# apache/yunikorn-k8shim

Measured on AMD Instinct MI355X. Metric: pod×node predicate evals/sec + decisions/sec, 50k nodes × 1M pods, higher is better.
Workload: dtype int64; 1 GPU; configs[2]: 50k nodes x 1M pods, NodeResourcesFit + TaintToleration + NodeAffinity; nodes_per_gpu=50000, total_nodes=50000, pods=1000000, templates=2000, pod_classes=2061, signature_planes=327, unique_requests=False, spread=False, gang_size=0, parallelism=single GPU

## Files before the change

### yunikorn-k8shim_amd/csrc/engine/engine.hip

```cpp
#include "../../../include/ykpred.h"

#include <hip/hip_runtime.h>
#include <dlfcn.h>
#include <rccl/rccl.h>

#include <algorithm>
#include <chrono>
#include <cstdio>
#include <cstdlib>
#include <cstring>
#include <mutex>
#include <string>
#include <map>
#include <unordered_map>
#include <vector>

#include "kernels.hip.h"
#include "ask_tasks.h"
#include "preempt_headroom_finish.h"

using ykk::i64;
using ykk::u64;

namespace {
// ... 230 lines not shown
  std::vector<uint8_t> vfx_stale;
  int64_t vfx_stale_nodes = 0;
  DevBuf d_pround_live;
  DevBuf d_bytes_gather;
  DevBuf d_topo_agree;
  u64 dict_digest = 0;
  int fuse_rows = 1;
  int fuse_wpl = 0;
  int fuse_count = 0, fuse_row_count = 0;
  bool fuse_ready = false;
  DevBuf d_fuse_rec;
  int fuse_combos = 0;
  int fuse_combine = 1;
  DevBuf d_fuse_combo_rec, d_fuse_combo;
  std::vector<uint8_t> h_class_fused;
  int run_decide = 1;
  int run_ranges = 0, n_decide_list = 0, run_decide_classes = -1;
  bool win_partial = false;
  DevBuf d_run_ranges, d_no_decide, d_glin_r;
  int class_runs = 1;
  int class_runs_min_rows = 16;
  int run_classes = 0, run_units = 0, run_rows = 0;
  DevBuf d_run_classes, d_run_units;
  DevBuf d_sweep_rows, d_sweep_runs, d_sweep_units;
  int sweep_units[ykk::kMaxIdxRows] = {0, 0}, sweep_unit_off[ykk::kMaxIdxRows + 1] = {0, 0, 0};
  DevBuf d_chunk_list_b0;
  int NCB0 = 0;
  DevBuf d_walk2_order, d_walk2_big, d_walk2_begin, d_walk2_len;
  int walk2_chunks = -1;
  DevBuf d_first_r;
  static constexpr bool decide_skip = true;
  DevBuf d_chunk_list_b;
  DevBuf d_slice_general;
  DevBuf d_slice_desc;
  DevBuf d_pfx_r;
  DevBuf d_idx_c;
  DevBuf d_win_r;
  int idx_stride = 0;
  DevBuf d_sig_tol, d_sig_tolflags, d_sig_ports, d_swanted;
  DevBuf d_sig_aff_flags, d_sig_aff_off, d_sig_aff_terms, d_sig_pre_off, d_sig_pre_terms;
  bool specs_set = false;

  int P = 0, C = 0, NC = 0;
  std::vector<int32_t> h_pod_spec, h_pod_pin;
  DevBuf d_pod_spec, d_pod_pin, d_pod_class;
  DevBuf d_class_sig, d_class_pin, d_class_first, d_class_word, d_chunk_class, d_chunk_begin, d_chunk_len, d_chunk_first, d_members;
  std::unordered_map<ClassKey, int32_t, ClassKeyHash> class_ids;
  std::vector<int32_t> h_pod_class, h_pod_slot;
  std::vector<int32_t> h_pod_row;
  int rows_total = 0, rows_a = 0, row_capacity = 0;
  DevBuf d_pod_row;
  bool bands_enabled = true;
  int band_steps = 0;
  int band_steps_now = 128;
  int round_batched = -1;
  int round_node_assume = 1;
  int round_prof = 0;
  int fail_after = 0;
  int sig_wpl = 0;
  int combine_slices = 1;
  int decide_groups_from = 16384;
  int early_counts = 1;
  int group_lds = -1;
  int group_scratch_mb = 256;
  int affinity_fill_waves = 0;
  int group_chunk_tasks = 0;
  int max_lds_bytes = 64 * 1024;
  int num_cus = 256;
  int n_bands = 0, n_band_steps = 0, n_classes_a = 0, n_fix_rows = 0;
  std::vector<int32_t> h_class_slot_a;
  DevBuf d_band_tab, d_class_rows_a, d_class_list_a, d_class_slot_a, d_fix_row, d_fix_slot, d_chunk_zone;
  DevBuf d_class_list_b;
  int n_classes_b = 0;
  std::vector<int32_t> h_ch_zone;
  std::vector<uint8_t> h_row_stale;
  std::vector<int32_t> h_class_sig, h_class_pin, h_class_first, h_class_live;
  std::vector<std::vector<int32_t>> h_class_chunks;
  std::vector<int32_t> h_members, h_ch_class, h_ch_begin, h_ch_len, h_ch_first;
  int patch_chunks = 0;
  bool rank_valid = false;
  uint64_t specs_version = 1, ranked_specs_version = 0, ranked_nodes_epoch = 0;
  unsigned ranked_pre = 0, ranked_filt = 0;
  bool ranked_has_first = false;
  DevBuf d_round;
  DevBuf d_fx_off, d_fx_cls, d_fx_cnt, d_fx_occ, d_sp_sig_of;
  uint64_t fx_version = 0;
  bool fx_contrib = false, fx_ports = false;
  std::vector<int32_t> h_fx_off;
  std::vector<int32_t> h_fx_cls;
  std::vector<int32_t> h_fx_cnt;
  std::vector<uint8_t> h_fx_occupies;
  DevBuf d_patches, d_rows, d_row_count, d_row_best;
  unsigned last_pre = 0, last_filt = 0;
  bool last_eval_valid = false;
  DevBuf d_class_count, d_class_best;
  bool pods_set = false, classes_dirty = true;
  int chunk_members = ykk::kChunkMembers;
  bool chunk_sorted = true;
  int combine_lds_bytes = 40000;

  DevBuf d_bitmap, d_counts, d_decisions, d_keys, d_scratch;
  void* last_bitmap = nullptr;
  int64_t last_bitmap_rows = 0;
  void *last_counts = nullptr, *last_decisions = nullptr, *last_keys = nullptr;

  hipStream_t aux_stream = nullptr;
  hipEvent_t ev_fork = nullptr, ev_planes = nullptr, ev_join = nullptr, ev_counts = nullptr, ev_zero = nullptr;
  hipStream_t peek_stream = nullptr;
  hipEvent_t ev_eval_done = nullptr;
  void* peek_pinned = nullptr;
  size_t peek_pinned_bytes = 0;

  struct GraphKey {
    uint64_t version;
    unsigned pre, filt, options;
    void *bitmap, *counts, *decisions, *keys;
    bool operator==(const GraphKey& o) const {
      return version == o.version && pre == o.pre && filt == o.filt && options == o.options && bitmap == o.bitmap && counts == o.counts &&
             decisions == o.decisions && keys == o.keys;
    }
  };
  std::vector<std::pair<GraphKey, hipGraphExec_t>> graphs;
  std::vector<GraphKey> seen;
  uint64_t tables_version = 1;
  bool graph_disabled = true;

  ncclComm_t comm = nullptr;
  int comm_rank = 0, comm_world = 1, node_offset = 0;
  int64_t round_exchanges = 0;
  void* h_round_pinned = nullptr;
  size_t h_round_pinned_bytes = 0;
  int64_t rounds_batched = 0, round_batched_asks = 0, round_batches = 0, rounds_sequential = 0, round_sequential_asks = 0;
  int forced_stride = 0;
  DevBuf d_gathered, d_gathered_map, d_xkey, d_xcand;
  bool last_has_keys = false;
  DevBuf d_class_rows_all, d_gathered_classes, d_class_rows_slot, d_class_sig_ident, d_expand_count, d_layout_hash, d_gathered_pod_class, d_row_pod;
  int ident_classes = 0;
  uint64_t layout_version = 1, layout_hashed_version = 0, layout_hash_value = 0, row_pod_version = 0;
  uint64_t ask_epoch = 1, hdr_epoch = 0;
  std::vector<uint64_t> hdr_cache;
  uint64_t nodes_epoch = 1, hist_epoch = 0;
  uint64_t bitmap_epoch = 0;

  int64_t n_full_evals = 0, n_node_patches = 0, n_row_patches = 0, n_queries = 0, n_gathers = 0, n_uploads = 0;

  hipEvent_t ev[2 * YKPRED_MAX_TIMED_KERNELS + 2]{};
  bool ev_ready = false;
  int timed = 0;
  const char* timed_name[YKPRED_MAX_TIMED_KERNELS]{};
  bool timing_valid = false;
};

namespace {

int fail(ykpred_engine* e, int code, const std::string& msg) {
  if (e) e->err = msg;
  if (e && (code == YKPRED_E_DEVICE || code == YKPRED_E_NOMEM)) {
    e->last_eval_valid = false;
    e->rank_valid = false;
    e->classes_dirty = true;
    e->spread_dirty = true;
    e->hist_epoch = 0;
    e->ranked_nodes_epoch = 0;
    e->tables_version++;
  }
  return code;
}
inline bool inject_failure(ykpred_engine* e) { return e && e->fail_after > 0 && --e->fail_after == 0; }
#define HIPCHK(call)                                                                                        \
  do {                                                                                                      \
    hipError_t _s = inject_failure(e) ? hipErrorUnknown : (call);                                          \
    if (_s != hipSuccess)                                                                                   \
      return fail(e, _s == hipErrorOutOfMemory ? YKPRED_E_NOMEM : YKPRED_E_DEVICE,                          \
                  std::string(#call) + ": " + hipGetErrorString(_s));                                       \
  } while (0)

template <class T>
int upload(ykpred_engine* e, DevBuf& b, const T* src, size_t n, hipStream_t st) {
  HIPCHK(b.ensure(n * sizeof(T)));
  if (n) HIPCHK(hipMemcpyAsync(b.p, src, n * sizeof(T), hipMemcpyHostToDevice, st));
  return YKPRED_OK;
}
#define TRY(x)                     \
  do {                             \
    int _r = (x);                  \
    if (_r != YKPRED_OK) return _r; \
  } while (0)

ykk::NodeTable node_table(const ykpred_engine* e) {
  ykk::NodeTable t;
  t.n = e->N;
  t.R = e->R;
  t.KT = e->KT;
  t.W = e->W;
  t.alloc = e->d_alloc.as<i64>();
  t.req = e->d_req.as<i64>();
  t.allowed = e->d_allowed.as<int>();
  t.count = e->d_count.as<int>();
  t.flags = e->d_nflags.as<unsigned>();
  t.taints = e->d_taints.as<u64>();
  t.labels = e->d_labels.as<u64>();
  t.KD = e->KD;
  t.KS = e->KS;
  t.domain = e->d_domain.as<int>();
  t.selcount = e->d_selcount.as<int>();
  t.KP = e->KP;
  t.ports = e->d_ports.as<u64>();
  return t;
}
ykk::SpreadSigs spread_sigs(const ykpred_engine* e) {
  ykk::SpreadSigs sp;
  sp.D = e->fam_spread.D;
  sp.c_off = e->d_sp_coff.as<int>();
  sp.c = e->d_sp_c.as<ykk::SpreadC>();
  sp.aff_sig = e->d_sp_aff.as<int>();
  sp.tol_sig = e->d_sp_tol.as<int>();
  sp.cnt = e->d_sp_cnt.as<int>();
  sp.present = e->d_sp_present.as<int>();
  sp.minv = e->d_sp_min.as<int>();
  return sp;
}
ykk::SpecTable spec_table(const ykpred_engine* e) {
  ykk::SpecTable s;
  s.R = e->R;
  s.KT = e->KT;
  s.W = e->W;
  s.req = e->d_sreq.as<i64>();
  s.tol = e->d_stol.as<u64>();
  s.flags = e->d_sflags.as<unsigned>();
  s.aff.flags = e->d_sflags.as<unsigned>();
  s.aff.term_off = e->d_aff_off.as<int>();
  s.aff.terms = e->d_aff_terms.as<u64>();
  s.aff.pre_off = e->d_pre_off.as<int>();
  s.aff.pre_terms = e->d_pre_terms.as<u64>();
  s.KP = e->KP;
  s.wanted_ports = e->d_swanted.as<u64>();
  s.spread_sig = e->d_spec_spread.as<int>();
  s.spread = spread_sigs(e);
  return s;
}

int build_classes(ykpred_engine* e, hipStream_t st) {
  e->tables_version++;
  const int P = e->P;
  auto& ids = e->class_ids;
  ids.clear();
  ids.reserve(1024);
  auto& pod_class = e->h_pod_class;
  pod_class.assign((size_t)P, 0);
  auto &class_sig = e->h_class_sig, &class_pin = e->h_class_pin, &class_size = e->h_class_live;
  class_sig.clear();
  class_pin.clear();
  class_size.clear();
  for (int p = 0; p < P; ++p) {
    int s = e->h_pod_spec[(size_t)p];
    ClassKey k{e->spec_sig_res[(size_t)s], e->spec_sig_tol[(size_t)s], e->spec_sig_aff[(size_t)s], e->spec_sig_spread[(size_t)s],
               e->h_pod_pin[(size_t)p]};
    auto it = ids.find(k);
    int32_t c;
    if (it == ids.end()) {
      c = (int32_t)class_pin.size();
      ids.emplace(k, c);
      class_sig.insert(class_sig.end(), {k.a, k.b, k.c, k.d});
      class_pin.push_back(k.pin);
      class_size.push_back(0);
    } else {
      c = it->second;
    }
    pod_class[(size_t)p] = c;
    class_size[(size_t)c]++;
  }
  const int C = (int)class_pin.size();
  std::vector<int32_t> class_off((size_t)C + 1, 0);
  for (int c = 0; c < C; ++c) class_off[(size_t)c + 1] = class_off[(size_t)c] + class_size[(size_t)c];
  auto& members = e->h_members;
  members.assign((size_t)P, 0);
  e->h_pod_slot.assign((size_t)P, 0);
  std::vector<int32_t> cursor(class_off.begin(), class_off.end() - 1);
  for (int p = 0; p < P; ++p) {
    int slot = cursor[(size_t)pod_class[(size_t)p]]++;
    members[(size_t)slot] = p;
    e->h_pod_slot[(size_t)p] = slot;
  }
  const long row_b = (long)e->row_stride * 8, win = (long)ykk::kBandGroups * 4096;
  const int KC = ykk::kBandClasses;
  auto piece_min_of = [&](int steps) { return (int)((double)steps * (4096.0 + (double)row_b) / (double)row_b / (double)(KC - 1) * 1.3) + 3; };
  int S = e->band_steps;
  if (S <= 0) {
    int s_min = 8;
    while (s_min < 128 && (long)s_min * 4096 < 5L * KC * row_b) s_min *= 2;
    auto coverage = [&](int steps) {
      const int need = 2 * piece_min_of(steps);
      long rows = 0;
      for (int c = 0; c < C; ++c)
        if (class_size[(size_t)c] >= need) rows += class_size[(size_t)c];
      return rows;
    };
    const long best = coverage(s_min);
    S = 128;
    while (S > s_min && (double)coverage(S) < 0.5 * (double)best) S /= 2;
  }
  while (S > 4 && (long)S * win / row_b >= (1L << 21)) S -= 4;
  e->band_steps_now = S;
  const int piece_min = piece_min_of(S);
  e->h_class_slot_a.assign((size_t)C, -1);
  e->h_pod_row.assign((size_t)P, -1);
  std::vector<ykk::BandEntry> band_tab;
  std::vector<int32_t> class_list_a, fix_row, fix_slot;
  int n_steps = 0, n_bands = 0, rows_a = 0;
  const bool geometry_ok = e->bands_enabled && e->N > 0 && (size_t)2 * KC * (size_t)row_b <= (size_t)std::min(ykk::kBandMaxLds, e->max_lds_bytes);
  if (geometry_ok) {
    long rows_needed = 0;
    for (int c = 0; c < C; ++c)
      if (class_size[(size_t)c] >= 2 * piece_min) {
        e->h_class_slot_a[(size_t)c] = (int32_t)class_list_a.size();
        class_list_a.push_back(c);
        rows_needed += class_size[(size_t)c];
      }
    if (rows_needed < (long)S * win / row_b / 4) {
      class_list_a.clear();
      std::fill(e->h_class_slot_a.begin(), e->h_class_slot_a.end(), -1);
    }
  }
  if (!class_list_a.empty()) {
    struct Piece {
      int32_t x, s, slot;
// ... 491 lines not shown
  if (e->row_capacity && e->rows_total > e->row_capacity)
    return fail(e, YKPRED_E_INVALID, "the bitmap needs more rows than ykpred_set_row_capacity allows");
  const int cm = e->chunk_members;
  struct Chunk {
    int32_t cls, begin, len, first, first_row;
  };
  std::vector<Chunk> chunks;
  for (int c = 0; c < C; ++c)
    for (int b = class_off[(size_t)c]; b < class_off[(size_t)c + 1]; b += cm)
      chunks.push_back({c, b, std::min(cm, class_off[(size_t)c + 1] - b), b == class_off[(size_t)c] ? 1 : 0, e->h_pod_row[(size_t)members[(size_t)b]]});
  if (e->chunk_sorted)
    std::stable_sort(chunks.begin(), chunks.end(), [](const Chunk& x, const Chunk& y) { return x.first_row < y.first_row; });
  auto &ch_class = e->h_ch_class, &ch_begin = e->h_ch_begin, &ch_len = e->h_ch_len, &ch_first = e->h_ch_first;
  ch_class.clear();
  ch_begin.clear();
  ch_len.clear();
  ch_first.clear();
  e->h_ch_zone.clear();
  e->h_class_chunks.assign((size_t)C, {});
  for (const Chunk& k : chunks) {
    e->h_class_chunks[(size_t)k.cls].push_back((int32_t)ch_class.size());
    ch_class.push_back(k.cls);
    ch_begin.push_back(k.begin);
    ch_len.push_back(k.len);
    ch_first.push_back(k.first);
    e->h_ch_zone.push_back(e->h_class_slot_a[(size_t)k.cls] >= 0 ? 1 : (e->h_class_sweep[(size_t)k.cls] ? 2 : (e->h_class_fused[(size_t)k.cls] ? 3 : 0)));
  }
  std::vector<int32_t> chunk_list_b;
  for (size_t k = 0; k < e->h_ch_zone.size(); ++k)
    if (e->h_ch_zone[k] != 1) chunk_list_b.push_back((int32_t)k);
  e->NCB = (int)chunk_list_b.size();
  {
    std::vector<int32_t> chunk_list_b0;
    for (size_t k = 0; k < e->h_ch_zone.size(); ++k)
      if (e->h_ch_zone[k] == 0) chunk_list_b0.push_back((int32_t)k);
    e->NCB0 = (int)chunk_list_b0.size();
    TRY(upload(e, e->d_chunk_list_b0, chunk_list_b0.data(), chunk_list_b0.size(), st));
  }
  e->h_class_first.assign((size_t)C, -1);
  for (int c = 0; c < C; ++c) e->h_class_first[(size_t)c] = members[(size_t)class_off[(size_t)c]];
  std::vector<int32_t> member_rows((size_t)P);
  for (int i = 0; i < P; ++i) member_rows[(size_t)i] = e->h_pod_row[(size_t)members[(size_t)i]];
  e->h_row_stale.assign((size_t)P, 0);
  e->C = C;
  e->NC = (int)ch_class.size();
  e->patch_chunks = 0;
  TRY(upload(e, e->d_pod_class, pod_class.data(), pod_class.size(), st));
  TRY(upload(e, e->d_class_sig, class_sig.data(), class_sig.size(), st));
  TRY(upload(e, e->d_class_pin, class_pin.data(), class_pin.size(), st));
  TRY(upload(e, e->d_class_first, e->h_class_first.data(), e->h_class_first.size(), st));
  TRY(upload(e, e->d_members, member_rows.data(), member_rows.size(), st));
  TRY(upload(e, e->d_pod_row, e->h_pod_row.data(), e->h_pod_row.size(), st));
  TRY(upload(e, e->d_chunk_zone, e->h_ch_zone.data(), e->h_ch_zone.size(), st));
  TRY(upload(e, e->d_chunk_list_b, chunk_list_b.data(), chunk_list_b.size(), st));
  TRY(upload(e, e->d_band_tab, band_tab.data(), band_tab.size(), st));
  TRY(upload(e, e->d_class_list_a, class_list_a.data(), class_list_a.size(), st));
  TRY(upload(e, e->d_class_slot_a, e->h_class_slot_a.data(), e->h_class_slot_a.size(), st));
  TRY(upload(e, e->d_fix_row, fix_row.data(), fix_row.size(), st));
  TRY(upload(e, e->d_fix_slot, fix_slot.data(), fix_slot.size(), st));
  HIPCHK(e->d_class_rows_a.ensure((size_t)std::max<size_t>(class_list_a.size(), 1) * (size_t)e->row_stride * sizeof(u64)));
  TRY(upload(e, e->d_chunk_class, ch_class.data(), ch_class.size(), st));
  TRY(upload(e, e->d_chunk_begin, ch_begin.data(), ch_begin.size(), st));
  TRY(upload(e, e->d_chunk_len, ch_len.data(), ch_len.size(), st));
  TRY(upload(e, e->d_chunk_first, ch_first.data(), ch_first.size(), st));
  HIPCHK(e->d_class_count.ensure((size_t)std::max(C, 1) * sizeof(int)));
  HIPCHK(e->d_class_best.ensure((size_t)std::max(C, 1) * sizeof(int)));
  HIPCHK(hipStreamSynchronize(st));
  e->classes_dirty = false;
  e->layout_version++;
  e->last_eval_valid = false;
  return YKPRED_OK;
}

int ensure_planes(ykpred_engine* e, hipStream_t st) {
  int rows = 0;
  for (Family* f : {&e->fam_res, &e->fam_spread, &e->fam_tol, &e->fam_aff}) {
    f->base = rows;
    rows += std::max(f->D, 1);
  }
  size_t need = ((size_t)rows * (size_t)e->row_stride + 64) * sizeof(u64);
  for (DevBuf* b : {&e->planes_canon, &e->planes_ranked}) {
    if (b->cap < need || e->plane_rows_alloc != rows) {
      e->tables_version++;
      HIPCHK(b->ensure(need));
      HIPCHK(hipMemsetAsync(b->p, 0, need, st));
    }
  }
  e->plane_rows_alloc = rows;
  size_t base_need = (size_t)(64 * (e->W + e->KT + e->KP) + 2) * (size_t)e->row_stride * sizeof(u64);
  for (DevBuf* b : {&e->base_canon, &e->base_ranked}) {
    if (b->cap < base_need) {
      e->tables_version++;
      HIPCHK(b->ensure(base_need));
      HIPCHK(hipMemsetAsync(b->p, 0, base_need, st));
    }
  }
  return YKPRED_OK;
}

int build_spread_tables(ykpred_engine* e, hipStream_t st) {
  e->tables_version++;
  std::vector<int32_t> coff{0}, aff, tol;
  std::vector<ykk::SpreadC> rows;
  int64_t cells = 0;
  for (size_t d = 0; d < e->spread_sig.size(); ++d) {
    for (const ykpred_spread_t& c : e->spread_sig[d]) {
      if (c.topology_key < 0 || c.topology_key >= e->KD || c.selector_class >= e->KS)
        return fail(e, YKPRED_E_INVALID, "spread constraint references a topology key / selector class outside the node table");
      ykk::SpreadC r;
      r.kd = c.topology_key;
      r.ks = c.selector_class;
      r.max_skew = c.max_skew;
      r.min_domains = c.min_domains;
      r.self_match = c.self_match;
      r.flags = c.flags;
      r.kind = c.kind;
      r.dom_size = (size_t)c.topology_key < e->h_domain_sizes.size() ? e->h_domain_sizes[(size_t)c.topology_key] : 0;
      r.cnt_off = (int)cells;
      cells += r.dom_size;
      if (cells > 0x7fffffff) return fail(e, YKPRED_E_UNSUPPORTED, "spread histograms exceed 2^31 cells");
      rows.push_back(r);
    }
    coff.push_back((int32_t)rows.size());
    aff.push_back(e->spread_sig_aff[d]);
    tol.push_back(e->spread_sig_tol[d]);
  }
  e->spread_constraints = (int)rows.size();
  e->spread_cells = cells;
  TRY(upload(e, e->d_sp_coff, coff.data(), coff.size(), st));
  TRY(upload(e, e->d_sp_c, rows.data(), rows.size(), st));
  TRY(upload(e, e->d_sp_aff, aff.data(), aff.size(), st));
  TRY(upload(e, e->d_sp_tol, tol.data(), tol.size(), st));
  {
    std::vector<int32_t> sig_of;
    for (size_t d = 0; d < e->spread_sig.size(); ++d) sig_of.insert(sig_of.end(), e->spread_sig[d].size(), (int32_t)d);
    sig_of.resize(std::max<size_t>(rows.size(), 1), 0);
    TRY(upload(e, e->d_sp_sig_of, sig_of.data(), sig_of.size(), st));
  }
  HIPCHK(e->d_sp_cnt.ensure((size_t)std::max<int64_t>(cells, 1) * sizeof(int)));
  HIPCHK(e->d_sp_present.ensure((size_t)std::max<int64_t>(cells, 1) * sizeof(int)));
  HIPCHK(e->d_sp_min.ensure((size_t)std::max(e->spread_constraints, 1) * sizeof(int)));
  HIPCHK(hipStreamSynchronize(st));
  e->spread_dirty = false;
  return YKPRED_OK;
}

struct Timer {
  ykpred_engine* e;
  bool on;
  void start(hipStream_t st) {
    e->timed = 0;
    e->timing_valid = false;
    if (on) (void)hipEventRecord(e->ev[2 * YKPRED_MAX_TIMED_KERNELS], st);
  }
  void begin(hipStream_t st) {
    if (on && e->timed < YKPRED_MAX_TIMED_KERNELS) (void)hipEventRecord(e->ev[2 * e->timed], st);
  }
  void end(hipStream_t st, const char* name) {
    if (trace_kernels_on()) {
      const hipError_t s = hipStreamSynchronize(st);
      fprintf(stderr, "ykpred: %s %s\n", name, s == hipSuccess ? "done" : hipGetErrorString(s));
      fflush(stderr);
    }
    if (!on || e->timed >= YKPRED_MAX_TIMED_KERNELS) return;
    (void)hipEventRecord(e->ev[2 * e->timed + 1], st);
    e->timed_name[e->timed] = name;
    e->timed++;
  }
  void done(hipStream_t st) {
    if (on) (void)hipEventRecord(e->ev[2 * YKPRED_MAX_TIMED_KERNELS + 1], st);
    e->timing_valid = on;
  }
};

int grow_owned_outputs(ykpred_engine* e) {
// ... 237 lines not shown
    g_create_error = "ABI version mismatch";
    return YKPRED_E_INVALID;
  }
  if (cfg->num_resources < 3 || cfg->num_resources > ykk::kMaxR || cfg->taint_words < 1 || cfg->taint_words > ykk::kMaxKT ||
      cfg->label_words < 1 || cfg->label_words > ykk::kMaxWTotal) {
    g_create_error = "config out of range: need 3<=R<=8, 1<=KT<=4, 1<=W<=32";
    return YKPRED_E_UNSUPPORTED;
  }
  if (cfg->topology_keys < 0 || cfg->topology_keys > ykk::kMaxKD || cfg->selector_classes < 0 || cfg->selector_classes > 4096 ||
      cfg->port_words < 0 || cfg->port_words > ykk::kMaxKP) {
    g_create_error = "config out of range: need 0<=KD<=8 topology keys, 0<=KS<=4096 selector classes, 0<=KP<=4 port words";
    return YKPRED_E_UNSUPPORTED;
  }
  int ndev = 0;
  hipError_t s = hipGetDeviceCount(&ndev);
  if (s != hipSuccess || ndev <= 0) {
    g_create_error = std::string("no HIP device: ") + hipGetErrorString(s) + " (libykpred has no CPU fallback)";
    return YKPRED_E_DEVICE;
  }
  if (cfg->device < 0 || cfg->device >= ndev) {
    g_create_error = "device ordinal out of range";
    return YKPRED_E_INVALID;
  }
  s = hipSetDevice(cfg->device);
  if (s != hipSuccess) {
    g_create_error = std::string("hipSetDevice: ") + hipGetErrorString(s);
    return YKPRED_E_DEVICE;
  }
  auto* e = new ykpred_engine();
  e->cfg = *cfg;
  e->R = cfg->num_resources;
  e->KT = cfg->taint_words;
  e->W = cfg->label_words;
  e->KD = cfg->topology_keys;
  e->KS = cfg->selector_classes;
  e->KP = cfg->port_words;
  if (cfg->reserved[0] >= 1 && cfg->reserved[0] <= ykk::kChunkMembers) e->chunk_members = cfg->reserved[0];
  e->chunk_sorted = cfg->reserved[1] != 1;
  if (cfg->reserved[2] > 0 && cfg->reserved[2] <= 160 * 1024) e->combine_lds_bytes = cfg->reserved[2];
  if (cfg->reserved[2] < 0) e->combine_lds_bytes = 0;
  if (cfg->reserved[4] > 0) e->walk_rows = cfg->reserved[4];
  if (cfg->reserved[5] > 0) e->wave_combine_below = cfg->reserved[5];
  if (cfg->reserved[5] < 0) e->wave_combine_below = 0;
  if (cfg->reserved[6] < 0) e->bands_enabled = false;
  if (cfg->reserved[6] > 0) e->band_steps = std::min(256, std::max(4, (cfg->reserved[6] + 3) / 4 * 4));
  e->graph_disabled = cfg->reserved[3] != 1;
  {
    int lds = 0;
    if (hipDeviceGetAttribute(&lds, hipDeviceAttributeMaxSharedMemoryPerBlock, cfg->device) == hipSuccess && lds > 0) e->max_lds_bytes = lds;
    int cus = 0;
    if (hipDeviceGetAttribute(&cus, hipDeviceAttributeMultiprocessorCount, cfg->device) == hipSuccess && cus > 0) e->num_cus = cus;
  }
  if (const char* tune = getenv("YKPRED_TUNE")) {
    std::string text(tune);
    size_t at = 0;
    while (at < text.size()) {
      size_t stop = text.find(',', at);
      if (stop == std::string::npos) stop = text.size();
      const std::string item = text.substr(at, stop - at);
      at = stop + 1;
      if (item.empty()) continue;
      const size_t eq = item.find('=');
      const std::string key = item.substr(0, eq);
      const int val = eq == std::string::npos ? 1 : atoi(item.c_str() + eq + 1);
      if (key == "walk_rows") e->walk_rows = std::max(val, 1);
      else if (key == "sig_wpl") e->sig_wpl = val;
      else if (key == "combine_slices") e->combine_slices = val;
      else if (key == "decide_groups_from") e->decide_groups_from = val;
      else if (key == "graph") e->graph_disabled = val != 1;
      else if (key == "early_counts") e->early_counts = val;
      else if (key == "band_steps") {
        e->bands_enabled = val >= 0;
        e->band_steps = val > 0 ? std::min(256, std::max(4, (val + 3) / 4 * 4)) : 0;
      } else if (key == "chunk_members") e->chunk_members = std::min(std::max(val, 1), (int)ykk::kChunkMembers);
      else if (key == "wave_combine_below") e->wave_combine_below = std::max(val, 0);
      else if (key == "fail_after") e->fail_after = std::max(val, 0);
      else if (key == "round_prof") e->round_prof = val;
      else if (key == "round_batched") e->round_batched = val;
      else if (key == "round_node_assume") e->round_node_assume = val;
      else if (key == "sweep_min_run") e->sweep_min_run = std::max(val, 0);
      else if (key == "sweep_groups") e->sweep_groups = std::max(val, 0);
      else if (key == "class_runs") e->class_runs = val;
      else if (key == "run_decide") e->run_decide = val;
      else if (key == "fuse_rows") e->fuse_rows = val;
      else if (key == "fuse_wpl") e->fuse_wpl = val;
      else if (key == "fuse_combine") e->fuse_combine = val;
      else if (key == "class_runs_min_rows") e->class_runs_min_rows = std::max(val, 1);
      else if (key == "group_lds") e->group_lds = val;
      else if (key == "group_scratch_mb") e->group_scratch_mb = std::max(val, 0);
      else if (key == "group_chunk_tasks") e->group_chunk_tasks = std::max(val, 0);
      else if (key == "affinity_fill_waves") e->affinity_fill_waves = val;
      else {
        g_create_error = "YKPRED_TUNE: unknown key '" + key + "'";
        delete e;
        return YKPRED_E_INVALID;
      }
    }
  }
  s = hipStreamCreateWithFlags(&e->own_stream, hipStreamNonBlocking);
  if (s != hipSuccess) {
    g_create_error = std::string("hipStreamCreate: ") + hipGetErrorString(s);
    delete e;
    return YKPRED_E_DEVICE;
  }
  {
    int lo = 0, hi = 0;
    (void)hipDeviceGetStreamPriorityRange(&lo, &hi);
    if (hipStreamCreateWithPriority(&e->aux_stream, hipStreamNonBlocking, hi) != hipSuccess)
      (void)hipStreamCreateWithFlags(&e->aux_stream, hipStreamNonBlocking);
  }
  if (hipStreamCreateWithFlags(&e->peek_stream, hipStreamNonBlocking) != hipSuccess) e->peek_stream = nullptr;
  (void)hipEventCreateWithFlags(&e->ev_eval_done, hipEventDisableTiming);
  (void)hipEventCreateWithFlags(&e->ev_fork, hipEventDisableTiming);
  (void)hipEventCreateWithFlags(&e->ev_join, hipEventDisableTiming);
  (void)hipEventCreateWithFlags(&e->ev_planes, hipEventDisableTiming);
  (void)hipEventCreateWithFlags(&e->ev_counts, hipEventDisableTiming);
  (void)hipEventCreateWithFlags(&e->ev_zero, hipEventDisableTiming);
  for (auto& ev : e->ev) (void)hipEventCreate(&ev);
  e->ev_ready = true;
  *out = e;
  return YKPRED_OK;
}

void ykpred_destroy(ykpred_engine_t* e) {
  if (!e) return;
  (void)hipSetDevice(e->cfg.device);
  (void)hipDeviceSynchronize();
  if (e->comm) (void)rccl()->CommDestroy(e->comm);
  e->comm = nullptr;
  for (DevBuf* b : {&e->d_gathered, &e->d_gathered_map, &e->d_xkey, &e->d_xcand}) b->release();
  for (auto& g : e->graphs) (void)hipGraphExecDestroy(g.second);
  e->graphs.clear();
  for (DevBuf* b : {&e->d_alloc, &e->d_req, &e->d_allowed, &e->d_count, &e->d_nflags, &e->d_taints, &e->d_labels, &e->d_domain, &e->d_selcount, &e->d_ports, &e->d_sig_ports, &e->d_swanted,
                    &e->d_sp_cnt_prev, &e->d_sp_present_prev, &e->d_sp_min_prev, &e->d_sig_changed, &e->d_class_dirty,
                    &e->d_spec_spread, &e->d_sp_coff, &e->d_sp_c, &e->d_sp_aff, &e->d_sp_tol, &e->d_sp_cnt, &e->d_sp_present, &e->d_sp_min,
                    &e->planes_canon, &e->planes_ranked, &e->base_canon, &e->base_ranked, &e->d_rankbuf, &e->d_score, &e->d_key,
                    &e->d_rank, &e->d_perm, &e->d_sreq, &e->d_stol, &e->d_sflags, &e->d_aff_off, &e->d_aff_terms, &e->d_pre_off,
                    &e->d_pre_terms, &e->d_dim_val, &e->d_dim_order, &e->d_dim_chunk_dim, &e->d_dim_chunk_begin, &e->d_dim_chunk_len,
                    &e->d_res_rows, &e->d_big_dim, &e->d_walk_big, &e->d_walk_begin, &e->d_walk_len, &e->d_sfree_c, &e->d_pmask_c,
                    &e->d_sfree_r, &e->d_pmask_r, &e->d_rbits_c, &e->d_sorted, &e->d_sorted_off, &e->d_ent_c, &e->d_agree, &e->d_topo_agree, &e->d_bytes_gather, &e->d_fuse_rec, &e->d_fuse_combo_rec, &e->d_fuse_combo, &e->d_run_ranges, &e->d_no_decide, &e->d_glin_r, &e->d_run_classes, &e->d_run_units, &e->d_sweep_rows, &e->d_sweep_runs, &e->d_sweep_units, &e->d_chunk_list_b0, &e->d_walk2_order, &e->d_walk2_big, &e->d_walk2_begin, &e->d_walk2_len, &e->d_idx_c, &e->d_win_r, &e->d_pfx_r, &e->d_slice_desc, &e->d_slice_general, &e->d_chunk_list_b, &e->d_first_r, &e->d_sig_tol, &e->d_sig_tolflags, &e->d_sig_aff_flags, &e->d_sig_aff_off,
                    &e->d_sig_aff_terms, &e->d_sig_pre_off, &e->d_sig_pre_terms, &e->d_pod_spec, &e->d_pod_pin, &e->d_pod_class,
                    &e->d_class_sig, &e->d_class_pin, &e->d_class_first, &e->d_class_word, &e->d_chunk_class, &e->d_chunk_begin, &e->d_chunk_len, &e->d_chunk_first,
                    &e->d_pod_row, &e->d_band_tab, &e->d_class_rows_a, &e->d_class_list_a, &e->d_class_slot_a, &e->d_fix_row, &e->d_fix_slot, &e->d_chunk_zone,
                    &e->d_members, &e->d_patches, &e->d_rows, &e->d_row_count, &e->d_row_best, &e->d_class_count, &e->d_class_best, &e->d_bitmap, &e->d_counts, &e->d_decisions, &e->d_keys, &e->d_scratch,
                    &e->d_member_key, &e->d_name_rank, &e->d_member_tie, &e->d_class_rows_all, &e->d_gathered_classes, &e->d_class_rows_slot,
                    &e->d_class_sig_ident, &e->d_expand_count, &e->d_layout_hash, &e->d_gathered_pod_class, &e->d_row_pod,
                    &e->d_round, &e->d_fx_off, &e->d_fx_cls, &e->d_fx_cnt, &e->d_fx_occ, &e->d_sp_sig_of, &e->d_class_list_b, &e->d_gathered, &e->d_gathered_map,
                    &e->d_xkey, &e->d_xcand, &e->d_query, &e->d_groups, &e->d_domain_head, &e->d_rc_req, &e->d_rc_pods, &e->d_rc_ports,
                    &e->d_vt_base, &e->d_vt_tier_end, &e->d_vt_cum, &e->d_vt_ports, &e->d_pround})
    b->release();
  if (e->ev_ready)
    for (auto& ev : e->ev) (void)hipEventDestroy(ev);
  if (e->ev_fork) (void)hipEventDestroy(e->ev_fork);
  if (e->ev_join) (void)hipEventDestroy(e->ev_join);
  if (e->ev_planes) (void)hipEventDestroy(e->ev_planes);
  if (e->ev_counts) (void)hipEventDestroy(e->ev_counts);
  if (e->ev_zero) (void)hipEventDestroy(e->ev_zero);
  if (e->h_round_pinned) (void)hipHostFree(e->h_round_pinned);
  if (e->ev_eval_done) (void)hipEventDestroy(e->ev_eval_done);
  if (e->peek_pinned) (void)hipHostFree(e->peek_pinned);
  if (e->peek_stream) (void)hipStreamDestroy(e->peek_stream);
  if (e->aux_stream) (void)hipStreamDestroy(e->aux_stream);
  if (e->own_stream) (void)hipStreamDestroy(e->own_stream);
  delete e;
}

int32_t ykpred_set_nodes(ykpred_engine_t* e, const ykpred_nodes_t* n) {
  YK_SERIALISE(e);
  Range roctx_range("ykpred:upload_nodes");
  if (e) e->n_uploads++;
  if (e) e->tables_version++;
  if (e) e->nodes_epoch++;
  if (e) e->ask_epoch++;
  if (e) e->last_eval_valid = false;
  if (!e || !n || n->count < 0) return fail(e, YKPRED_E_INVALID, "set_nodes: bad argument");
  if (n->count > 0 && (!n->allocatable || !n->requested || !n->allowed_pods || !n->pod_count || !n->flags || !n->taint_bits ||
                       !n->label_bits))
    return fail(e, YKPRED_E_INVALID, "set_nodes: null column");
  if ((e->KD > 0 && (!n->domain_sizes || (n->count > 0 && !n->domain_id))) || (e->KS > 0 && n->count > 0 && !n->selector_count))
    return fail(e, YKPRED_E_INVALID, "set_nodes: topology / selector columns missing (config has KD/KS > 0)");
  if (e->KP > 0 && n->count > 0 && !n->port_bits) return fail(e, YKPRED_E_INVALID, "set_nodes: port_bits missing (config has KP > 0)");
  HIPCHK(hipSetDevice(e->cfg.device));
  hipStream_t st = e->own_stream;
  e->rank_valid = false;
  const size_t N = (size_t)n->count;
  TRY(upload(e, e->d_alloc, n->allocatable, N * (size_t)e->R, st));
  TRY(upload(e, e->d_req, n->requested, N * (size_t)e->R, st));
  TRY(upload(e, e->d_allowed, n->allowed_pods, N, st));
  TRY(upload(e, e->d_count, n->pod_count, N, st));
  TRY(upload(e, e->d_nflags, n->flags, N, st));
  TRY(upload(e, e->d_taints, n->taint_bits, N * (size_t)e->KT, st));
  TRY(upload(e, e->d_labels, n->label_bits, N * (size_t)e->W, st));
  TRY(upload(e, e->d_domain, n->domain_id, N * (size_t)e->KD, st));
  TRY(upload(e, e->d_selcount, n->selector_count, N * (size_t)e->KS, st));
  TRY(upload(e, e->d_ports, n->port_bits, N * (size_t)e->KP, st));
  e->has_name_rank = n->name_rank != nullptr && N > 0;
  if (e->has_name_rank) TRY(upload(e, e->d_name_rank, n->name_rank, N, st));
  HIPCHK(e->d_member_tie.ensure(std::max<size_t>(N, 1) * sizeof(int)));
  for (int k = 0; k < ykk::kMaxKT; ++k) e->taint_used[k] = 0;
  for (int k = 0; k < e->KT; ++k)
    for (size_t i = 0; i < N; ++i) e->taint_used[k] |= n->taint_bits[(size_t)k * N + i];
  e->h_domain_sizes.assign(n->domain_sizes, n->domain_sizes + e->KD);
  e->spread_dirty = true;
  HIPCHK(e->d_score.ensure(N * sizeof(double)));
  HIPCHK(e->d_key.ensure(N * sizeof(u64)));
  HIPCHK(e->d_rank.ensure(N * sizeof(int)));
  HIPCHK(e->d_perm.ensure(N * sizeof(int)));
  HIPCHK(e->d_rankbuf.ensure((3 * (size_t)ykk::kRankBuckets + 1 + N) * sizeof(int)));
  HIPCHK(e->d_member_key.ensure(N * sizeof(u64)));
  HIPCHK(hipStreamSynchronize(st));
  if (e->N != n->count) {
    e->planes_canon.release();
    e->planes_ranked.release();
    e->base_canon.release();
    e->base_ranked.release();
    e->rc_tiers = 0;
    e->vt_tiers = 0;
    e->vfx_columns = -1;
  }
  e->N = n->count;
  e->row_words = (e->N + 63) / 64;
  e->row_stride = std::max(16, (e->row_words + 15) / 16 * 16);
  if (e->forced_stride) {
    if (e->forced_stride < e->row_stride) return fail(e, YKPRED_E_INVALID, "set_nodes: ykpred_set_row_stride is smaller than this shard needs");
    e->row_stride = e->forced_stride;
  }
  e->nodes_set = true;
  return YKPRED_OK;
}

int32_t ykpred_update_node(ykpred_engine_t* e, int32_t idx, const ykpred_nodes_t* n) {
  YK_SERIALISE(e);
  Range roctx_range("ykpred:update_node");
  if (e) e->n_uploads++;
  if (e) e->tables_version++;
  if (!e || !n || n->count != 1) return fail(e, YKPRED_E_INVALID, "update_node: count must be 1");
  if (!e->nodes_set || idx < 0 || idx >= e->N) return fail(e, YKPRED_E_INVALID, "update_node: index out of range");
  for (int k = 0; k < e->KD; ++k)
    if (n->domain_id[k] >= e->h_domain_sizes[(size_t)k]) return fail(e, YKPRED_E_INVALID, "update_node: new topology domain — re-upload the node table");
  e->nodes_epoch++;
  HIPCHK(hipSetDevice(e->cfg.device));
  hipStream_t st = e->own_stream;
  e->rank_valid = false;
  const size_t N = (size_t)e->N;
  for (int r = 0; r < e->R; ++r) {
    HIPCHK(hipMemcpyAsync(e->d_alloc.as<i64>() + (size_t)r * N + idx, n->allocatable + r, sizeof(i64), hipMemcpyHostToDevice, st));
    HIPCHK(hipMemcpyAsync(e->d_req.as<i64>() + (size_t)r * N + idx, n->requested + r, sizeof(i64), hipMemcpyHostToDevice, st));
  }
  HIPCHK(hipMemcpyAsync(e->d_allowed.as<int>() + idx, n->allowed_pods, sizeof(int), hipMemcpyHostToDevice, st));
  HIPCHK(hipMemcpyAsync(e->d_count.as<int>() + idx, n->pod_count, sizeof(int), hipMemcpyHostToDevice, st));
  HIPCHK(hipMemcpyAsync(e->d_nflags.as<unsigned>() + idx, n->flags, sizeof(unsigned), hipMemcpyHostToDevice, st));
  for (int k = 0; k < e->KT; ++k) {
    e->taint_used[k] |= n->taint_bits[k];
    HIPCHK(hipMemcpyAsync(e->d_taints.as<u64>() + (size_t)k * N + idx, n->taint_bits + k, sizeof(u64), hipMemcpyHostToDevice, st));
  }
  for (int w = 0; w < e->W; ++w)
    HIPCHK(hipMemcpyAsync(e->d_labels.as<u64>() + (size_t)w * N + idx, n->label_bits + w, sizeof(u64), hipMemcpyHostToDevice, st));
  for (int k = 0; k < e->KD; ++k) {
    HIPCHK(hipMemcpyAsync(e->d_domain.as<int>() + (size_t)k * N + idx, n->domain_id + k, sizeof(int), hipMemcpyHostToDevice, st));
  }
  for (int k = 0; k < e->KS; ++k)
    HIPCHK(hipMemcpyAsync(e->d_selcount.as<int>() + (size_t)k * N + idx, n->selector_count + k, sizeof(int), hipMemcpyHostToDevice, st));
  for (int k = 0; k < e->KP; ++k)
    HIPCHK(hipMemcpyAsync(e->d_ports.as<u64>() + (size_t)k * N + idx, n->port_bits + k, sizeof(u64), hipMemcpyHostToDevice, st));
  if (e->has_name_rank && n->name_rank)
    HIPCHK(hipMemcpyAsync(e->d_name_rank.as<int>() + idx, n->name_rank, sizeof(int), hipMemcpyHostToDevice, st));
  HIPCHK(hipStreamSynchronize(st));
  return YKPRED_OK;
}

int32_t ykpred_update_label_word(ykpred_engine_t* e, int32_t word, const uint64_t* column) {
  YK_SERIALISE(e);
  if (!e || !column || word < 0 || word >= (e ? e->W : 0)) return fail(e, YKPRED_E_INVALID, "update_label_word: bad argument");
  if (!e->nodes_set) return fail(e, YKPRED_E_STATE, "update_label_word: no node table");
  e->tables_version++;
  HIPCHK(hipSetDevice(e->cfg.device));
  if (e->N) {
    HIPCHK(hipMemcpyAsync(e->d_labels.as<u64>() + (size_t)word * (size_t)e->N, column, (size_t)e->N * sizeof(u64), hipMemcpyHostToDevice, e->own_stream));
    HIPCHK(hipStreamSynchronize(e->own_stream));
  }
  return YKPRED_OK;
}

int32_t ykpred_set_specs(ykpred_engine_t* e, const ykpred_specs_t* s) {
  YK_SERIALISE(e);
  Range roctx_range("ykpred:upload_specs");
  if (e) e->n_uploads++;
  if (e) e->tables_version++;
  if (e) e->ask_epoch++;
  if (e) e->specs_version++;
  if (!e || !s || s->count < 0) return fail(e, YKPRED_E_INVALID, "set_specs: bad argument");
  if (s->count > 0 && (!s->requests || !s->tolerated || !s->flags || !s->aff_term_off || !s->pre_term_off))
    return fail(e, YKPRED_E_INVALID, "set_specs: null column");
  if (s->spread_off && s->count > 0 && s->spread_off[s->count] != 0 && !s->spread)
    return fail(e, YKPRED_E_INVALID, "set_specs: spread_off without spread rows");
  HIPCHK(hipSetDevice(e->cfg.device));
  hipStream_t st = e->own_stream;
  const int S = s->count, R = e->R, KT = e->KT, W = e->W, KP = e->KP;
  if (KP > 0 && S > 0 && !s->wanted_ports) return fail(e, YKPRED_E_INVALID, "set_specs: wanted_ports missing (config has KP > 0)");
  const int T = S ? s->aff_term_off[S] : 0, M = S ? s->pre_term_off[S] : 0;
  if (T < 0 || M < 0 || (T > 0 && !s->aff_terms) || (M > 0 && !s->pre_terms)) return fail(e, YKPRED_E_INVALID, "set_specs: bad term tables");
  const int oldS = e->S, old_spread_D = e->fam_spread.D;
  bool append_only = e->specs_set && !e->classes_dirty && oldS <= S;
  if (append_only && oldS > 0) {
    auto same = [](const void* a, const void* b, size_t n) { return n == 0 || memcmp(a, b, n) == 0; };
    const int oT = e->h_aff_off[(size_t)oldS], oM = e->h_pre_off[(size_t)oldS];
    append_only = same(e->h_req.data(), s->requests, (size_t)oldS * R * sizeof(i64)) &&
                  same(e->h_tol.data(), s->tolerated, (size_t)oldS * KT * sizeof(u64)) &&
                  (KP == 0 || same(e->h_wanted.data(), s->wanted_ports, (size_t)oldS * KP * sizeof(u64))) &&
                  same(e->h_sflags.data(), s->flags, (size_t)oldS * sizeof(uint32_t)) &&
                  same(e->h_aff_off.data(), s->aff_term_off, (size_t)(oldS + 1) * sizeof(int32_t)) &&
                  same(e->h_pre_off.data(), s->pre_term_off, (size_t)(oldS + 1) * sizeof(int32_t)) &&
                  same(e->h_aff_terms.data(), s->aff_terms, (size_t)oT * W * sizeof(u64)) &&
                  same(e->h_pre_terms.data(), s->pre_terms, (size_t)oM * W * sizeof(u64));
    const bool had_spread = !e->h_spread_off.empty() && e->h_spread_off[(size_t)oldS] > 0;
    if (append_only && (had_spread || s->spread_off)) {
      if (e->h_spread_off.empty() || !s->spread_off) {
        append_only = !had_spread && s->spread_off && s->spread_off[oldS] == 0;
      } else {
        append_only = same(e->h_spread_off.data(), s->spread_off, (size_t)(oldS + 1) * sizeof(int32_t)) &&
                      same(e->h_spread.data(), s->spread, (size_t)e->h_spread_off[(size_t)oldS] * sizeof(ykpred_spread_t));
      }
    }
  }
  if (s->spread_off && S > 0) {
    e->h_spread_off.assign(s->spread_off, s->spread_off + S + 1);
    e->h_spread.assign(s->spread, s->spread + s->spread_off[S]);
  } else {
    e->h_spread_off.assign((size_t)S + 1, 0);
    e->h_spread.clear();
  }
  e->S = S;
  e->h_req.assign(s->requests, s->requests + (size_t)S * R);
  e->h_tol.assign(s->tolerated, s->tolerated + (size_t)S * KT);
  if (KP > 0) e->h_wanted.assign(s->wanted_ports, s->wanted_ports + (size_t)S * KP); else e->h_wanted.clear();
  TRY(upload(e, e->d_swanted, e->h_wanted.data(), e->h_wanted.size(), st));
  e->h_sflags.assign(s->flags, s->flags + S);
  e->h_aff_off.assign(s->aff_term_off, s->aff_term_off + S + (S ? 1 : 0));
  e->h_pre_off.assign(s->pre_term_off, s->pre_term_off + S + (S ? 1 : 0));
  if (!S) {
    e->h_aff_off.assign(1, 0);
    e->h_pre_off.assign(1, 0);
  }
  e->h_aff_terms.assign(s->aff_terms, s->aff_terms + (size_t)T * W);
  e->h_pre_terms.assign(s->pre_terms, s->pre_terms + (size_t)M * W);
  TRY(upload(e, e->d_sreq, e->h_req.data(), e->h_req.size(), st));
  TRY(upload(e, e->d_stol, e->h_tol.data(), e->h_tol.size(), st));
  TRY(upload(e, e->d_sflags, e->h_sflags.data(), e->h_sflags.size(), st));
  TRY(upload(e, e->d_aff_off, e->h_aff_off.data(), e->h_aff_off.size(), st));
  TRY(upload(e, e->d_pre_off, e->h_pre_off.data(), e->h_pre_off.size(), st));
  TRY(upload(e, e->d_aff_terms, e->h_aff_terms.data(), e->h_aff_terms.size(), st));
  TRY(upload(e, e->d_pre_terms, e->h_pre_terms.data(), e->h_pre_terms.size(), st));

  e->spec_sig_res.assign((size_t)S, 0);
  e->spec_sig_tol.assign((size_t)S, 0);
  e->spec_sig_aff.assign((size_t)S, 0);
  std::unordered_map<std::string, int32_t> m_tol, m_aff;
  auto mix64 = [](u64 z) {
    z = (z ^ (z >> 30)) * 0xbf58476d1ce4e5b9ull;
    z = (z ^ (z >> 27)) * 0x94d049bb133111ebull;
    return z ^ (z >> 31);
  };
  size_t tab_cap = 64;
  while (tab_cap < (size_t)S * 2 + 2) tab_cap <<= 1;
  std::vector<int32_t> res_tab(tab_cap, -1);
  std::vector<int32_t> res_first;
  std::vector<std::vector<int32_t>> dim_tab((size_t)R);
  std::vector<size_t> dim_used((size_t)R, 0);
  auto dim_row = [&](int r, i64 q) -> int32_t {
    std::vector<int32_t>& tab = dim_tab[(size_t)r];
    if (tab.empty()) tab.assign(1024, -1);
    if ((dim_used[(size_t)r] + 1) * 2 > tab.size()) {
      std::vector<int32_t> bigger(tab.size() * 4, -1);
// ... 152 lines not shown
      std::vector<int32_t> big_of_dim((size_t)R, 0);
      for (size_t b = 0; b < big_dim.size(); ++b) big_of_dim[(size_t)big_dim[b]] = (int32_t)b + 1;
      for (int32_t& r : res_rows)
        if (r > 0 && big_of_dim[(size_t)e->h_dim_of[(size_t)r]]) r |= big_of_dim[(size_t)e->h_dim_of[(size_t)r]] << ykk::kRowBigShift;
    }
    e->index_rows = 0;
    for (int32_t len : wlen) e->index_rows += len;
    e->h_res_rows = res_rows;
    e->h_row_pos.assign((size_t)rows, -1);
    e->h_row_big.assign((size_t)rows, -1);
    e->sweep_ready = false;
    e->h_sorted_off.assign(1, 0);
    {
      std::vector<i64> sorted;
      for (size_t b = 0; b < big_dim.size(); ++b) {
        const int g = big_dim[b] + 1, b0 = start[(size_t)g], b1 = start[(size_t)g + 1];
        for (int i = b0; i < b1; ++i) {
          e->h_row_pos[(size_t)order[(size_t)i]] = i - b0;
          e->h_row_big[(size_t)order[(size_t)i]] = (int32_t)b;
          sorted.push_back(e->h_dim_val[(size_t)order[(size_t)i]]);
        }
        e->h_sorted_off.push_back((int32_t)sorted.size());
      }
      sorted.push_back(0);
      TRY(upload(e, e->d_sorted, sorted.data(), sorted.size(), st));
      TRY(upload(e, e->d_sorted_off, e->h_sorted_off.data(), e->h_sorted_off.size(), st));
    }
    e->h_stage_rows.clear();
    {
      std::vector<uint8_t> walked((size_t)R, 0);
      for (int32_t d : big_dim) walked[(size_t)d] = 1;
      for (int d = 1; d < rows && (int)e->h_stage_rows.size() < ykk::kWalkMaxStage; ++d)
        if (!walked[(size_t)e->h_dim_of[(size_t)d]]) e->h_stage_rows.push_back(d);
    }
    e->dim_chunks = (int)cdim.size();
    e->n_big = (int)big_dim.size();
    e->walk_chunks = (int)wbig.size();
    TRY(upload(e, e->d_dim_val, e->h_dim_val.data(), e->h_dim_val.size(), st));
    TRY(upload(e, e->d_dim_order, order.data(), order.size(), st));
    TRY(upload(e, e->d_dim_chunk_dim, cdim.data(), cdim.size(), st));
    TRY(upload(e, e->d_dim_chunk_begin, cbegin.data(), cbegin.size(), st));
    TRY(upload(e, e->d_dim_chunk_len, clen.data(), clen.size(), st));
    TRY(upload(e, e->d_big_dim, big_dim.data(), big_dim.size(), st));
    TRY(upload(e, e->d_walk_big, wbig.data(), wbig.size(), st));
    TRY(upload(e, e->d_walk_begin, wbegin.data(), wbegin.size(), st));
    TRY(upload(e, e->d_walk_len, wlen.data(), wlen.size(), st));
    TRY(upload(e, e->d_res_rows, res_rows.data(), res_rows.size(), st));
  }
  TRY(upload(e, e->d_sig_tol, sig_tol.data(), sig_tol.size(), st));
  TRY(upload(e, e->d_sig_tolflags, sig_tolflags.data(), sig_tolflags.size(), st));
  TRY(upload(e, e->d_sig_ports, sig_ports.data(), sig_ports.size(), st));
  TRY(upload(e, e->d_sig_aff_flags, sig_aff_flags.data(), sig_aff_flags.size(), st));
  TRY(upload(e, e->d_sig_aff_off, sig_aff_off.data(), sig_aff_off.size(), st));
  TRY(upload(e, e->d_sig_pre_off, sig_pre_off.data(), sig_pre_off.size(), st));
  TRY(upload(e, e->d_sig_aff_terms, sig_aff_terms.data(), sig_aff_terms.size(), st));
  TRY(upload(e, e->d_sig_pre_terms, sig_pre_terms.data(), sig_pre_terms.size(), st));
  HIPCHK(hipStreamSynchronize(st));
  e->specs_set = true;
  if (!append_only) e->classes_dirty = true;
  if (!spread_unchanged) e->last_eval_valid = false;
  return YKPRED_OK;
}

int32_t ykpred_set_pods(ykpred_engine_t* e, const ykpred_pods_t* p) {
  YK_SERIALISE(e);
  Range roctx_range("ykpred:upload_asks");
  if (e) e->n_uploads++;
  if (e) e->tables_version++;
  if (e) e->ask_epoch++;
  if (!e || !p || p->count < 0) return fail(e, YKPRED_E_INVALID, "set_pods: bad argument");
  if (p->count > 0 && (!p->spec_index || !p->node_name_index)) return fail(e, YKPRED_E_INVALID, "set_pods: null column");
  HIPCHK(hipSetDevice(e->cfg.device));
  e->P = p->count;
  e->h_pod_spec.assign(p->spec_index, p->spec_index + p->count);
  e->h_pod_pin.assign(p->node_name_index, p->node_name_index + p->count);
  TRY(upload(e, e->d_pod_spec, e->h_pod_spec.data(), e->h_pod_spec.size(), e->own_stream));
  TRY(upload(e, e->d_pod_pin, e->h_pod_pin.data(), e->h_pod_pin.size(), e->own_stream));
  HIPCHK(hipStreamSynchronize(e->own_stream));
  e->pods_set = true;
  e->classes_dirty = true;
  return YKPRED_OK;
}

static int validate_state(ykpred_engine* e) {
  if (!e->nodes_set || !e->specs_set || !e->pods_set) return fail(e, YKPRED_E_STATE, "nodes, specs and pods must be uploaded first");
  for (int p = 0; p < e->P; ++p) {
    int s = e->h_pod_spec[(size_t)p], pin = e->h_pod_pin[(size_t)p];
    if (s < 0 || s >= e->S) return fail(e, YKPRED_E_INVALID, "pod references a spec that was not uploaded");
    if (pin < YKPRED_UNKNOWN_NODE_NAME || pin >= e->N) return fail(e, YKPRED_E_INVALID, "pod node_name_index out of range");
  }
  return YKPRED_OK;
}

int32_t ykpred_eval(ykpred_engine_t* e, const ykpred_eval_args_t* a) {
  YK_SERIALISE(e);
  Range roctx_range("ykpred:eval");
  if (!e || !a) return fail(e, YKPRED_E_INVALID, "eval: bad argument");
  HIPCHK(hipSetDevice(e->cfg.device));
  hipStream_t st = a->stream ? (hipStream_t)a->stream : e->own_stream;
  if (e->classes_dirty) {
    if (a->options & (YKPRED_EVAL_SKIP_BITMAP | YKPRED_EVAL_DIRTY_CLASSES))
      return fail(e, YKPRED_E_STATE, "eval: the pod classes are due for a rebuild — run a full ykpred_eval (bitmap included)");
    TRY(validate_state(e));
    TRY(build_classes(e, e->own_stream));
  }
  const unsigned pre = a->prefilter_plugins, filt = a->filter_plugins;
  const bool spread_filt = filt & YKPRED_PLUGIN_POD_TOPOLOGY_SPREAD, spread_pre = pre & YKPRED_PLUGIN_POD_TOPOLOGY_SPREAD;
  const bool ipa_filt = filt & YKPRED_PLUGIN_INTER_POD_AFFINITY, ipa_pre = pre & YKPRED_PLUGIN_INTER_POD_AFFINITY;
  const bool spread_err = (spread_filt && !spread_pre) || (ipa_filt && !ipa_pre) ||
                          ((filt & YKPRED_PLUGIN_NODE_PORTS) && !(pre & YKPRED_PLUGIN_NODE_PORTS));
  if (e->spread_dirty) TRY(build_spread_tables(e, e->own_stream));
  const bool pts_en = spread_filt && spread_pre, ipa_en = ipa_filt && ipa_pre;
  const bool spread_on = (pts_en || ipa_en) && e->fam_spread.D > 0;
  const int N = e->N, P = e->P;
  const size_t bitmap_bytes = (size_t)std::max(std::max(e->rows_total, e->row_capacity), 1) * (size_t)e->row_stride * sizeof(u64);
  u64* bitmap = (u64*)a->bitmap;
  int64_t bitmap_rows = 0;
  if (!bitmap || (void*)bitmap == e->d_bitmap.p) {
    HIPCHK(e->d_bitmap.ensure(bitmap_bytes));
    bitmap = e->d_bitmap.as<u64>();
    bitmap_rows = (int64_t)(e->d_bitmap.cap / ((size_t)std::max(e->row_stride, 1) * sizeof(u64)));
  } else {
    bitmap_rows = a->bitmap_rows ? (int64_t)a->bitmap_rows : (int64_t)e->row_capacity;
    if (bitmap_rows == 0)
      return fail(e, YKPRED_E_INVALID, "eval: a caller-owned bitmap needs eval_args.bitmap_rows or ykpred_set_row_capacity (it must hold layout.num_rows rows)");
    if ((int64_t)e->rows_total > bitmap_rows)
      return fail(e, YKPRED_E_INVALID, "eval: the caller-owned bitmap holds fewer rows than the layout needs (layout.num_rows)");
  }
  e->last_bitmap = bitmap;
  e->last_bitmap_rows = bitmap_rows;
  HIPCHK(e->d_counts.ensure((size_t)std::max(P, 1) * sizeof(int)));
  HIPCHK(e->d_decisions.ensure((size_t)std::max(P, 1) * sizeof(int)));
  HIPCHK(e->d_keys.ensure((size_t)std::max(P, 1) * sizeof(i64)));
  e->last_counts = a->counts ? a->counts : e->d_counts.p;
  e->last_decisions = a->decisions ? a->decisions : e->d_decisions.p;
  e->last_keys = a->decision_keys ? a->decision_keys : e->d_keys.p;
  TRY(ensure_planes(e, st));
  if (e->n_big > 0) {
    const size_t cells = (size_t)e->n_big * (size_t)std::max(e->row_words, 1);
    for (DevBuf* b : {&e->d_sfree_c, &e->d_sfree_r}) HIPCHK(b->ensure(cells * 64 * sizeof(i64)));
    for (DevBuf* b : {&e->d_pmask_c, &e->d_pmask_r}) HIPCHK(b->ensure(cells * 65 * sizeof(u64)));
    HIPCHK(e->d_rbits_c.ensure(cells * ykk::kRankBits * sizeof(u64)));
    HIPCHK(e->d_ent_c.ensure(cells * 65 * sizeof(unsigned)));
    HIPCHK(e->d_glin_r.ensure(cells * 65 * sizeof(unsigned)));
    const int idx_stride_before = e->idx_stride;
    e->idx_stride = (std::max(e->row_words, e->row_stride) + 63) / 64 * 64;
    for (DevBuf* b : {&e->d_idx_c}) {
      const size_t need = (size_t)e->fam_res.D * (size_t)e->idx_stride;
      if (b->cap < need || !b->p || idx_stride_before != e->idx_stride) {
        HIPCHK(b->ensure(need));
        HIPCHK(hipMemsetAsync(b->p, 64, need, st));
      }
    }
    {
      const size_t need = (size_t)e->fam_res.D * 64;
      if (e->d_win_r.cap < need || !e->d_win_r.p) {
        HIPCHK(e->d_win_r.ensure(need));
        HIPCHK(hipMemsetAsync(e->d_win_r.p, 64, need, st));
      }
    }
  }
  Timer tm{e, (a->options & YKPRED_EVAL_PROFILE) != 0};
  tm.start(st);
  if (N == 0 || P == 0) {
    tm.done(st);
    return YKPRED_OK;
  }
  ykk::NodeTable nt = node_table(e);
  const bool want_keys = a->options & YKPRED_OUT_DECISION_KEYS;
  const bool want_dec = (a->options & YKPRED_OUT_DECISIONS) || want_keys;
  const bool want_cnt = a->options & YKPRED_OUT_COUNTS;
  const int nblk_nodes = (N + ykk::kBlock - 1) / ykk::kBlock;

  bool use_run_decide_pass = false;
  auto enqueue = [&]() -> int {
  if (spread_on || (a->options & YKPRED_EVAL_SPREAD_COUNT_ONLY)) {
    const bool ready = a->options & YKPRED_EVAL_SPREAD_COUNTS_READY, only = a->options & YKPRED_EVAL_SPREAD_COUNT_ONLY;
    TRY(run_spread_prefilter(e, st, &tm, !ready, false));
    if (only) return 1;
    if (!ready) TRY(allreduce_spread(e, st));
    TRY(run_spread_prefilter(e, st, &tm, false, true));
    e->hist_epoch = e->nodes_epoch;
  }
  if (a->options & YKPRED_EVAL_DIRECT) {
    ykk::SpecTable stbl = spec_table(e);
    dim3 grid((unsigned)((P + ykk::kWave - 1) / ykk::kWave), (unsigned)((e->row_stride + ykk::kWavesPerBlock - 1) / ykk::kWavesPerBlock));
    tm.begin(st);
    hipLaunchKernelGGL(ykk::k_direct, grid, dim3(ykk::kBlock), 0, st, nt, stbl, P, e->d_pod_spec.as<int>(), e->d_pod_pin.as<int>(),
                       e->d_pod_row.as<int>(), pre, filt, bitmap, e->row_words, e->row_stride);
    tm.end(st, "k_direct");
    HIPCHK(hipGetLastError());
    return 1;
  }

  const unsigned wgroups = (unsigned)((e->row_words + ykk::kWavesPerBlock - 1) / ykk::kWavesPerBlock);
  const bool res_on = filt & YKPRED_PLUGIN_NODE_RESOURCES_FIT;
  const bool aff_on = (filt | pre) & YKPRED_PLUGIN_NODE_AFFINITY;
  const int fit_error = (pre & YKPRED_PLUGIN_NODE_RESOURCES_FIT) ? 0 : 1;
  auto sig_chunks = [](int D) {
    const int spb = ykk::sigs_per_block(D);
    return (unsigned)((D + spb - 1) / spb);
  };
  ykk::AffSigs as{e->d_sig_aff_flags.as<unsigned>(), e->d_sig_aff_off.as<int>(), e->d_sig_aff_terms.as<u64>(), e->d_sig_pre_off.as<int>(),
                  e->d_sig_pre_terms.as<u64>()};
  auto canon_of = [&](const Family& f) { return e->planes_canon.as<u64>() + (size_t)f.base * e->row_stride; };
  auto ranked_of = [&](const Family& f) { return e->planes_ranked.as<u64>() + (size_t)f.base * e->row_stride; };
  ykk::PlaneOut o_res{canon_of(e->fam_res), ranked_of(e->fam_res), e->row_stride, e->fam_res.D, nullptr};
  ykk::PlaneOut o_tol{canon_of(e->fam_tol), ranked_of(e->fam_tol), e->row_stride, e->fam_tol.D, nullptr};
  ykk::PlaneOut o_aff{canon_of(e->fam_aff), ranked_of(e->fam_aff), e->row_stride, e->fam_aff.D, nullptr};
  ykk::PlaneOut o_spread{canon_of(e->fam_spread), ranked_of(e->fam_spread), e->row_stride, e->fam_spread.D, nullptr};
  const bool full_pass = !(a->options & (YKPRED_EVAL_SKIP_BITMAP | YKPRED_EVAL_DIRTY_CLASSES));
  const bool counts_early_here = e->early_counts != 0 && full_pass && e->n_classes_a > 0 && e->patch_chunks == 0 &&
                                 !((long)e->NC * e->wave_combine_below > (long)P) && e->n_classes_b <= 16384;
  const bool zero_counts_beside = full_pass && !counts_early_here && e->ev_zero != nullptr && e->C >= 65536 &&
                                  (a->options & (YKPRED_OUT_DECISIONS | YKPRED_OUT_DECISION_KEYS)) != 0;
  const bool use_sweep = e->sweep_ready && e->sweep_runs > 0 && res_on && !fit_error && full_pass && !counts_early_here;
  const bool sweep_rows_on = use_sweep && e->n_big > 0 && e->sweep_row_off[ykk::kMaxIdxRows] > 0;
  const bool fuse_on = e->fuse_ready && res_on && !fit_error && full_pass && !counts_early_here && aff_on && !spread_err;
  const bool use_run_decide = e->run_decide != 0 && e->sweep_ready && e->run_ranges > 0 && res_on && !fit_error && e->n_big > 0 &&
                              (a->options & (YKPRED_OUT_DECISIONS | YKPRED_OUT_DECISION_KEYS)) && e->walk2_chunks >= 0 &&
                              e->C == e->run_decide_classes;
  use_run_decide_pass = use_run_decide;
  ykk::ClassTable ct{e->d_class_sig.as<int>(), e->d_class_pin.as<int>(),  e->d_chunk_class.as<int>(), e->d_chunk_begin.as<int>(),
                     e->d_chunk_len.as<int>(), e->d_chunk_first.as<int>(), e->d_members.as<int>(), e->d_chunk_zone.as<int>(), (use_sweep ? 1 : 0) | (fuse_on ? 2 : 0),
                     use_run_decide ? e->d_no_decide.as<int>() : nullptr};
  ykk::Planes pc{res_on ? o_res.canon : nullptr, o_tol.canon, aff_on ? o_aff.canon : nullptr, spread_on ? o_spread.canon : nullptr,
                 e->row_stride, e->d_res_rows.as<int>(), 1 + e->R, e->d_idx_c.as<unsigned char>(), e->idx_stride, e->d_pmask_c.as<u64>(), e->row_words,
                 nullptr, 0, 0, 0, 0, 0, nullptr, nullptr, nullptr, nullptr, nullptr};
  int* first_r = nullptr;
  if ((a->options & (YKPRED_OUT_DECISIONS | YKPRED_OUT_DECISION_KEYS)) && e->decide_skip) {
    HIPCHK(e->d_first_r.ensure((size_t)std::max(e->plane_rows_alloc, 1) * sizeof(int)));
    first_r = e->d_first_r.as<int>();
  }
  if (want_dec && res_on && e->n_big > 0 && !fit_error) HIPCHK(e->d_pfx_r.ensure((size_t)e->n_big * (size_t)std::max(e->row_words, 1) * sizeof(i64)));
  ykk::Planes pr = ranked_planes_of(e, pre, filt, spread_on, first_r != nullptr);
  pc.n_big = pr.n_big;
  pc.rbits = e->d_rbits_c.as<u64>();
  const int pin_on = ((filt & YKPRED_PLUGIN_NODE_NAME) ? 1 : 0) | (spread_err ? 2 : 0);
  hipStream_t sb = e->aux_stream;

  if (want_dec) {
    HIPCHK(hipEventRecord(e->ev_fork, st));
    HIPCHK(hipStreamWaitEvent(sb, e->ev_fork, 0));
    if (zero_counts_beside) {
      HIPCHK(hipMemsetAsync(e->d_class_count.p, 0, (size_t)e->C * sizeof(int), sb));
      HIPCHK(hipEventRecord(e->ev_zero, sb));
    }
    if (first_r) HIPCHK(hipMemsetAsync(first_r, 0x7f, (size_t)std::max(e->plane_rows_alloc, 1) * sizeof(int), sb));
    tm.begin(sb);
    hipLaunchKernelGGL(ykk::k_score, dim3((unsigned)nblk_nodes), dim3(ykk::kBlock), 0, sb, nt, e->d_score.as<double>(), e->d_key.as<u64>());
    tm.end(sb, "k_score");
    int* hist = e->d_rankbuf.as<int>();
    int* bucket_off = hist + ykk::kRankBuckets;
    int* cursor = bucket_off + ykk::kRankBuckets + 1;
    int* members = cursor + ykk::kRankBuckets;
    HIPCHK(hipMemsetAsync(hist, 0, ykk::kRankBuckets * sizeof(int), sb));
    tm.begin(sb);
    hipLaunchKernelGGL(ykk::k_rank_hist, dim3((unsigned)nblk_nodes), dim3(ykk::kBlock), 0, sb, N, e->d_score.as<double>(), hist);
    hipLaunchKernelGGL(ykk::k_rank_scan, dim3(1), dim3(ykk::kRankBuckets), 0, sb, hist, bucket_off, cursor);
    hipLaunchKernelGGL(ykk::k_rank_fill, dim3((unsigned)nblk_nodes), dim3(ykk::kBlock), 0, sb, N, e->d_score.as<double>(), e->d_key.as<u64>(),
                       e->has_name_rank ? e->d_name_rank.as<int>() : (const int*)nullptr, cursor, members, e->d_member_tie.as<int>(),
                       e->d_member_key.as<u64>());
    hipLaunchKernelGGL(ykk::k_rank_final, dim3((unsigned)ykk::kRankBuckets), dim3(ykk::kBlock), 0, sb, bucket_off, members,
                       e->d_member_tie.as<int>(), e->d_member_key.as<u64>(), e->d_rank.as<int>(), e->d_perm.as<int>());
    tm.end(sb, "k_rank");
  }
  auto base_of = [&](DevBuf& buf) {
    ykk::BasePlanes bp;
    bp.req = buf.as<u64>();
    bp.taint = bp.req + (size_t)64 * e->W * e->row_stride;
    bp.port = bp.taint + (size_t)64 * e->KT * e->row_stride;
    bp.unsched = bp.port + (size_t)64 * e->KP * e->row_stride;
    bp.exists = bp.unsched + e->row_stride;
    bp.stride = e->row_stride;
    return bp;
  };
  auto launch_dictionary_planes = [&](hipStream_t s, const int* perm, bool ranked, const char* base_name, const char* sig_name, bool base_done = false) -> int {
    ykk::BasePlanes bp = base_of(ranked ? e->base_ranked : e->base_canon);
    if (!base_done) {
      tm.begin(s);
      hipLaunchKernelGGL(ykk::k_base_planes, dim3((unsigned)(e->W + e->KT + e->KP + 1), wgroups), dim3(ykk::kBlock), 0, s, nt, perm, bp,
                         e->row_words);
      tm.end(s, base_name);
    }
    ykk::SigPlaneArgs sa{};
    sa.base = bp;
    sa.tol = o_tol;
    sa.aff = o_aff;
    if (ranked) {
      sa.tol.canon = o_tol.ranked;
      sa.aff.canon = o_aff.ranked;
      sa.tol.first = first_r ? first_r + e->fam_tol.base : nullptr;
      sa.aff.first = first_r ? first_r + e->fam_aff.base : nullptr;
    }
    if (!aff_on) sa.aff.D = 0;
    sa.sig_tol = e->d_sig_tol.as<u64>();
    sa.sig_tolflags = e->d_sig_tolflags.as<unsigned>();
    sa.sig_ports = e->d_sig_ports.as<u64>();
    sa.KP = e->KP;
    for (int k = 0; k < ykk::kMaxKT; ++k) sa.taint_used[k] = e->taint_used[k];
    sa.affs = as;
    sa.KT = e->KT;
    sa.W = e->W;
    sa.pre_mask = pre;
    sa.filt_mask = filt;
    sa.n_words = e->row_words;
    tm.begin(s);
    const int wpl = e->sig_wpl > 0 ? e->sig_wpl : (e->row_words >= 4 * ykk::kWave ? 4 : (e->row_words >= 2 * ykk::kWave ? 2 : 1));
    const unsigned chunks = std::max((unsigned)((std::max(sa.tol.D, sa.aff.D) + ykk::kBitSigsPerBlock - 1) / ykk::kBitSigsPerBlock), 1u);
    const unsigned ygroups = (unsigned)((e->row_words + ykk::kBlock * wpl - 1) / (ykk::kBlock * wpl));
    if (wpl >= 4)
      hipLaunchKernelGGL(ykk::k_sig_planes<4>, dim3(chunks, ygroups, 2u), dim3(ykk::kBlock), 0, s, sa);
    else if (wpl >= 2)
      hipLaunchKernelGGL(ykk::k_sig_planes<2>, dim3(chunks, ygroups, 2u), dim3(ykk::kBlock), 0, s, sa);
    else
      hipLaunchKernelGGL(ykk::k_sig_planes<1>, dim3(chunks, ygroups, 2u), dim3(ykk::kBlock), 0, s, sa);
    tm.end(s, sig_name);
    return YKPRED_OK;
  };
  if (want_dec) TRY(launch_dictionary_planes(sb, e->d_perm.as<int>(), true, "k_base_planes(ranked)", "k_sig_planes(ranked)"));
  auto ranked_walk = [](const int* perm) { return perm != nullptr; };
  auto launch_ballot_planes = [&](hipStream_t s, const int* perm, const char* name, bool with_base = false) {
    ykk::PlaneArgs pa{};
    pa.perm = perm;
    pa.res = o_res;
    pa.spread = o_spread;
    if (perm && first_r) {
      pa.res.first = first_r + e->fam_res.base;
      pa.spread.first = first_r + e->fam_spread.base;
    }
    if (!spread_on) pa.spread.D = 0;
    pa.dims = ykk::DimPlanes{e->d_dim_val.as<i64>(), e->d_dim_order.as<int>(), e->d_dim_chunk_dim.as<int>(), e->d_dim_chunk_begin.as<int>(),
                             e->d_dim_chunk_len.as<int>(), res_on ? e->dim_chunks : 0};
    pa.spreads = spread_sigs(e);
    pa.fit_error = fit_error;
    pa.n_words = e->row_words;
    pa.spread_en = pts_en ? 1 : 0;
    pa.ipa_en = ipa_en ? 1 : 0;
    unsigned xchunks = std::max((unsigned)pa.dims.n_chunks, sig_chunks(pa.spread.D));
    tm.begin(s);
    if (with_base) {
      xchunks = std::max(xchunks, (unsigned)(e->W + e->KT + e->KP + 1));
      hipLaunchKernelGGL(ykk::k_node_planes, dim3(std::max(xchunks, 1u), wgroups, 3u), dim3(ykk::kBlock), 0, s, nt, pa,
                         base_of(perm ? e->base_ranked : e->base_canon));
    } else {
      hipLaunchKernelGGL(ykk::k_planes, dim3(std::max(xchunks, 1u), wgroups, spread_on ? 2u : 1u), dim3(ykk::kBlock), 0, s, nt, pa);
    }
    tm.end(s, name);
    if (res_on && e->n_big > 0 && !fit_error) {
      const bool ranked = perm != nullptr;
      ykk::DimWalk dw{e->d_dim_val.as<i64>(), e->d_dim_order.as<int>(), e->d_big_dim.as<int>(), e->d_walk_big.as<int>(), e->d_walk_begin.as<int>(),
                      e->d_walk_len.as<int>(), (ranked ? e->d_sfree_r : e->d_sfree_c).as<i64>(), (ranked ? e->d_pmask_r : e->d_pmask_c).as<u64>(),
                      e->n_big, e->walk_chunks, e->row_words, ranked ? nullptr : e->d_rbits_c.as<u64>(),
                      (!ranked && sweep_rows_on) ? e->d_ent_c.as<unsigned>() : nullptr, e->d_sorted.as<i64>(), e->d_sorted_off.as<int>(),
                      (ranked && use_run_decide) ? e->d_glin_r.as<unsigned>() : nullptr};
      tm.begin(s);
      hipLaunchKernelGGL(ykk::k_dim_sort, dim3((unsigned)e->n_big, wgroups), dim3(ykk::kBlock), 0, s, nt, perm, dw);
      tm.end(s, ranked ? "k_dim_sort(ranked)" : "k_dim_sort");
      tm.begin(s);
      const unsigned walk_gy = (unsigned)((e->row_words + ykk::kBlock * ykk::kWalkWords - 1) / (ykk::kBlock * ykk::kWalkWords));
      const dim3 walk_grid((unsigned)e->walk_chunks, walk_gy);
      if (!ranked && use_sweep && e->walk2_chunks >= 0) {
        if (e->walk2_chunks > 0) {
          ykk::DimWalk dw2 = dw;
          dw2.order = e->d_walk2_order.as<int>();
          dw2.chunk_big = e->d_walk2_big.as<int>();
          dw2.chunk_begin = e->d_walk2_begin.as<int>();
          dw2.chunk_len = e->d_walk2_len.as<int>();
          dw2.n_chunks = e->walk2_chunks;
          hipLaunchKernelGGL(ykk::k_dim_walk, dim3((unsigned)e->walk2_chunks, walk_gy), dim3(ykk::kBlock), 0, s, dw2, e->d_idx_c.as<unsigned char>(), e->idx_stride);
        }
      } else if (!ranked) {
        hipLaunchKernelGGL(ykk::k_dim_walk, walk_grid, dim3(ykk::kBlock), 0, s, dw, e->d_idx_c.as<unsigned char>(), e->idx_stride);
      } else {
        hipLaunchKernelGGL(ykk::k_dim_prefix_max, dim3((unsigned)e->n_big), dim3(ykk::kPfxBlock), 0, s, dw, e->d_pfx_r.as<i64>());
        if (use_run_decide) {
          if (e->walk2_chunks > 0) {
            ykk::DimWalk dw2 = dw;
            dw2.order = e->d_walk2_order.as<int>();
            dw2.chunk_big = e->d_walk2_big.as<int>();
            dw2.chunk_begin = e->d_walk2_begin.as<int>();
            dw2.chunk_len = e->d_walk2_len.as<int>();
            dw2.n_chunks = e->walk2_chunks;
            hipLaunchKernelGGL(ykk::k_dim_walk_window<8>, dim3((unsigned)e->walk2_chunks, walk_gy), dim3(ykk::kBlock), 0, s, dw2, e->d_pfx_r.as<i64>(), e->d_win_r.as<unsigned char>());
          }
        } else {
          hipLaunchKernelGGL(ykk::k_dim_walk_window<ykk::kWalkBatch>, walk_grid, dim3(ykk::kBlock), 0, s, dw, e->d_pfx_r.as<i64>(), e->d_win_r.as<unsigned char>());
        }
      }
      tm.end(s, ranked ? "k_dim_walk(ranked)" : "k_dim_walk");
    } else if (res_on && e->n_big > 0) {
      if (!ranked_walk(perm)) (void)hipMemsetAsync(e->d_idx_c.p, 64, (size_t)e->fam_res.D * (size_t)e->idx_stride, s);
      (void)hipMemsetAsync((ranked_walk(perm) ? e->d_pmask_r : e->d_pmask_c).p, 0, (size_t)e->n_big * (size_t)e->row_words * 65 * sizeof(u64), s);
      if (!ranked_walk(perm)) (void)hipMemsetAsync(e->d_rbits_c.p, 0, (size_t)e->n_big * (size_t)e->row_words * ykk::kRankBits * sizeof(u64), s);
    }
  };
  const bool fused_planes = res_on || spread_on;
  if (fused_planes) launch_ballot_planes(st, nullptr, "k_planes+k_base_planes", true);
  TRY(launch_dictionary_planes(st, nullptr, false, "k_base_planes", "k_sig_planes", fused_planes));
  if (want_dec) {
    HIPCHK(hipEventRecord(e->ev_planes, st));
    HIPCHK(hipStreamWaitEvent(sb, e->ev_planes, 0));
    const int ballot_rows = e->fam_tol.base;
    if (ballot_rows <= ykk::kManySigs && e->n_big == 0) {
      tm.begin(sb);
      hipLaunchKernelGGL(ykk::k_permute_planes, dim3(sig_chunks(ballot_rows), wgroups), dim3(ykk::kBlock), 0, sb, N, e->d_perm.as<int>(),
                         e->planes_canon.as<u64>(), e->planes_ranked.as<u64>(), e->row_stride, ballot_rows, e->row_words, first_r);
      tm.end(sb, "k_permute_planes");
    } else if (res_on || spread_on) {
      launch_ballot_planes(sb, e->d_perm.as<int>(), "k_planes(ranked)");
    }
    if (use_run_decide) {
      tm.begin(sb);
      hipLaunchKernelGGL(ykk::k_run_decide, dim3((unsigned)((e->run_ranges + ykk::kWavesPerBlock - 1) / ykk::kWavesPerBlock)), dim3(ykk::kBlock), 0, sb, pr,
                         e->d_sweep_runs.as<ykk::SweepRun>(), e->d_run_ranges.as<ykk::RunRange>(), e->run_ranges, e->d_sweep_rows.as<ykk::SweepRow>(),
                         e->d_glin_r.as<unsigned>(), e->d_sorted.as<i64>(), e->d_sorted_off.as<int>(), e->d_perm.as<int>(), e->row_words, N, pin_on,
                         e->d_class_best.as<int>());
      tm.end(sb, "k_run_decide");
    }
    tm.begin(sb);
    const int n_decide = use_run_decide ? e->n_decide_list : e->C;
    if (n_decide == 0) {
    } else if (n_decide >= e->decide_groups_from) {
      const int per_block = ykk::kWavesPerBlock * ykk::kDecideGroups;
      hipLaunchKernelGGL(ykk::k_decide_groups, dim3((unsigned)((n_decide + per_block - 1) / per_block)), dim3(ykk::kBlock), 0, sb, ct, pr, n_decide,
                         e->row_words, e->d_perm.as<int>(), e->d_rank.as<int>(), pin_on, e->d_class_best.as<int>());
    } else {
      hipLaunchKernelGGL(ykk::k_decide, dim3((unsigned)((n_decide + ykk::kWavesPerBlock - 1) / ykk::kWavesPerBlock)), dim3(ykk::kBlock), 0, sb, ct,
                         pr, n_decide, e->row_words, e->d_perm.as<int>(), e->d_rank.as<int>(), pin_on, e->d_class_best.as<int>(), n_decide <= 4096 ? 1 : 0);
    }
    tm.end(sb, "k_decide");
  }
  const bool skip_combine = a->options & YKPRED_EVAL_SKIP_BITMAP;
  const bool dirty_only = a->options & YKPRED_EVAL_DIRTY_CLASSES;
  const int* class_dirty = nullptr;
  if (!skip_combine && dirty_only) {
    HIPCHK(e->d_class_dirty.ensure((size_t)std::max(e->C, 1) * sizeof(int)));
    hipLaunchKernelGGL(ykk::k_mark_dirty_classes, dim3((unsigned)((e->C + ykk::kBlock - 1) / ykk::kBlock)), dim3(ykk::kBlock), 0, st, e->C,
                       e->d_class_sig.as<int>(), e->d_sig_changed.as<int>(), e->d_class_dirty.as<int>(), e->d_class_count.as<int>());
    class_dirty = e->d_class_dirty.as<int>();
  }
  const bool small_chunks = (long)e->NC * e->wave_combine_below > (long)P;
  const bool counts_early = e->early_counts != 0 && !skip_combine && !dirty_only && e->n_classes_a > 0 && e->patch_chunks == 0 && !small_chunks && e->n_classes_b <= 16384;
  bool scattered = false;
  if (!skip_combine && !dirty_only && !counts_early) {
    if (zero_counts_beside) HIPCHK(hipStreamWaitEvent(st, e->ev_zero, 0));
    else HIPCHK(hipMemsetAsync(e->d_class_count.p, 0, (size_t)e->C * sizeof(int), st));
  }
  if (!skip_combine) {
    int tpg = ykk::kBlock;
    while (tpg > ykk::kWave && (tpg / 2) * 2 >= e->row_stride) tpg /= 2;
    const int seg = tpg * ykk::kCombineUnroll * 2;
    const bool listed = !dirty_only && e->patch_chunks == 0;
    const bool short_list = use_sweep && (fuse_on || e->fuse_count == 0);
    const int* chunk_list = listed ? (short_list ? e->d_chunk_list_b0 : e->d_chunk_list_b).as<int>() : nullptr;
    const int n_run = listed ? (short_list ? e->NCB0 : e->NCB) : e->NC;
    dim3 grid((unsigned)std::max(n_run, 1), (unsigned)((e->row_stride + seg - 1) / seg));
    hipStream_t sz = st;
    if (!dirty_only && e->n_classes_a > 0) {
      tm.begin(st);
      const int n_counted_b = counts_early ? e->n_classes_b : 0;
      hipLaunchKernelGGL(ykk::k_class_rows, dim3((unsigned)((e->n_classes_a + n_counted_b + ykk::kWavesPerBlock - 1) / ykk::kWavesPerBlock)), dim3(ykk::kBlock), 0, st,
                         ct, pc, e->d_class_list_a.as<int>(), e->n_classes_a, e->row_words, e->row_stride, pin_on, e->d_class_rows_a.as<u64>(),
                         e->d_class_count.as<int>(), (const int*)nullptr, e->d_class_list_b.as<int>(), n_counted_b);
      tm.end(st, "k_class_rows");
      if (counts_early && want_dec) {
        HIPCHK(hipEventRecord(e->ev_counts, st));
        HIPCHK(hipStreamWaitEvent(sb, e->ev_counts, 0));
        tm.begin(sb);
        hipLaunchKernelGGL(ykk::k_scatter, dim3((unsigned)((P + ykk::kBlock - 1) / ykk::kBlock)), dim3(ykk::kBlock), 0, sb, P,
                           e->d_pod_class.as<int>(), e->d_class_count.as<int>(), e->d_class_best.as<int>(), e->d_key.as<u64>(),
                           want_cnt ? (int*)e->last_counts : nullptr, (int*)e->last_decisions, want_keys ? (i64*)e->last_keys : nullptr);
        tm.end(sb, "k_scatter");
        scattered = true;
      }
      const size_t lds_bytes = (size_t)2 * ykk::kBandClasses * (size_t)e->row_stride * sizeof(u64);
      if (lds_bytes > 64 * 1024)
        HIPCHK(hipFuncSetAttribute((const void*)ykk::k_expand_bands, hipFuncAttributeMaxDynamicSharedMemorySize, (int)lds_bytes));
      tm.begin(st);
      hipLaunchKernelGGL(ykk::k_expand_bands, dim3((unsigned)ykk::kBandGroups), dim3(ykk::kBandBlock), lds_bytes, st, bitmap,
                         e->d_class_rows_a.as<u64>(), e->d_band_tab.as<ykk::BandEntry>(), e->n_bands, e->row_stride);
      if (e->n_fix_rows > 0 && !counts_early)
        hipLaunchKernelGGL(ykk::k_fix_rows, dim3((unsigned)e->n_fix_rows), dim3(ykk::kBlock), 0, st, bitmap, e->d_class_rows_a.as<u64>(),
                           e->d_fix_row.as<int>(), e->d_fix_slot.as<int>(), e->n_fix_rows, e->row_stride);
      tm.end(st, "k_expand_bands");
    }
    if (use_sweep && e->run_classes > 0) {
      ykk::WalkStage rstage{};
      rstage.n = (int)e->h_stage_rows.size();
      for (int k = 0; k < rstage.n; ++k) rstage.row[k] = e->h_stage_rows[(size_t)k];
      const int its = (e->row_stride + ykk::kWave - 1) / ykk::kWave;
      int segs = (its + ykk::kWalkMaxIt - 1) / ykk::kWalkMaxIt, nit = (its + segs - 1) / segs;
      while (nit > 1 && ykk::runs_lds_bytes(rstage.n, nit) > (size_t)e->max_lds_bytes) {
        ++segs;
        nit = (its + segs - 1) / segs;
      }
      const int n_long = segs - (nit * segs - its);
      const size_t lds = ykk::runs_lds_bytes(rstage.n, nit);
      const int per_cu = lds * 2 <= (size_t)e->max_lds_bytes ? 2 : 1;
      const int groups = std::max(1, std::min(per_cu * e->num_cus, (e->run_units + ykk::kRunsWaves - 1) / ykk::kRunsWaves));
      tm.begin(sz);
      auto launch_runs = [&](auto kernel) -> int {
        if (lds > 64 * 1024) HIPCHK(hipFuncSetAttribute((const void*)kernel, hipFuncAttributeMaxDynamicSharedMemorySize, (int)lds));
        hipLaunchKernelGGL(kernel, dim3((unsigned)groups, (unsigned)segs), dim3(ykk::kRunsThreads), lds, sz, pc, e->d_run_classes.as<ykk::RunClass>(),
                           e->d_sweep_runs.as<ykk::SweepRun>(), e->run_classes, e->d_run_units.as<int>(), e->run_units, bitmap, e->row_words,
                           e->row_stride, pin_on, e->d_class_count.as<int>(), n_long, rstage);
        return YKPRED_OK;
      };
      switch (nit) {
        case 1: TRY(launch_runs(ykk::k_class_runs<1>)); break;
        case 2: TRY(launch_runs(ykk::k_class_runs<2>)); break;
        case 3: TRY(launch_runs(ykk::k_class_runs<3>)); break;
        case 4: TRY(launch_runs(ykk::k_class_runs<4>)); break;
        case 5: TRY(launch_runs(ykk::k_class_runs<5>)); break;
        case 6: TRY(launch_runs(ykk::k_class_runs<6>)); break;
        default: TRY(launch_runs(ykk::k_class_runs<7>)); break;
      }
      tm.end(sz, "k_class_runs");
    }
    if (sweep_rows_on) {
      const int its = (e->row_stride + ykk::kWave - 1) / ykk::kWave;
      int segs = (its + ykk::kWalkMaxIt - 1) / ykk::kWalkMaxIt, nit = (its + segs - 1) / segs;
      while (nit > 1 && ykk::sweep_lds_bytes(nit) > (size_t)e->max_lds_bytes) {
        ++segs;
        nit = (its + segs - 1) / segs;
      }
      const int n_long = segs - (nit * segs - its);
      tm.begin(sz);
      for (int b = 0; b < e->n_big; ++b) {
        const int n_rows = e->sweep_rows[b];
        if (n_rows == 0) continue;
        const int n_units = e->sweep_units[b];
        const int groups = std::max(1, std::min(e->sweep_groups > 0 ? e->sweep_groups : e->num_cus, (n_units + ykk::kSweepWaves - 1) / ykk::kSweepWaves));
        auto launch_sweep = [&](auto kernel) -> int {
          const size_t lds = ykk::sweep_lds_bytes(nit);
          if (lds > 64 * 1024) HIPCHK(hipFuncSetAttribute((const void*)kernel, hipFuncAttributeMaxDynamicSharedMemorySize, (int)lds));
          hipLaunchKernelGGL(kernel, dim3((unsigned)groups, (unsigned)segs), dim3(ykk::kSweepThreads), lds, sz, pc,
                             e->d_ent_c.as<unsigned>() + (size_t)b * 65 * (size_t)e->row_words, e->d_rbits_c.as<u64>() + (size_t)b * ykk::kRankBits * (size_t)e->row_words,
                             e->d_sweep_rows.as<ykk::SweepRow>() + e->sweep_row_off[b], e->d_sweep_runs.as<ykk::SweepRun>(), n_rows,
                             e->d_sweep_units.as<int>() + e->sweep_unit_off[b], n_units, bitmap, e->row_words, e->row_stride, pin_on,
                             e->d_class_count.as<int>(), n_long);
          return YKPRED_OK;
        };
        switch (nit) {
          case 1: TRY(launch_sweep(ykk::k_sweep_rows<1>)); break;
          case 2: TRY(launch_sweep(ykk::k_sweep_rows<2>)); break;
          case 3: TRY(launch_sweep(ykk::k_sweep_rows<3>)); break;
          case 4: TRY(launch_sweep(ykk::k_sweep_rows<4>)); break;
          case 5: TRY(launch_sweep(ykk::k_sweep_rows<5>)); break;
          case 6: TRY(launch_sweep(ykk::k_sweep_rows<6>)); break;
          default: TRY(launch_sweep(ykk::k_sweep_rows<7>)); break;
// ... 105 lines not shown
    HIPCHK(hipEventRecord(e->ev_join, sb));
    HIPCHK(hipStreamWaitEvent(st, e->ev_join, 0));
  }
  if ((want_dec || want_cnt) && !scattered) {
    tm.begin(st);
    hipLaunchKernelGGL(ykk::k_scatter, dim3((unsigned)((P + ykk::kBlock - 1) / ykk::kBlock)), dim3(ykk::kBlock), 0, st, P,
                       e->d_pod_class.as<int>(), e->d_class_count.as<int>(), e->d_class_best.as<int>(), e->d_key.as<u64>(),
                       want_cnt ? (int*)e->last_counts : nullptr, want_dec ? (int*)e->last_decisions : nullptr,
                       want_keys ? (i64*)e->last_keys : nullptr);
    tm.end(st, "k_scatter");
  }
  HIPCHK(hipGetLastError());
  return YKPRED_OK;
  };
  const bool graphable = !tm.on && !e->graph_disabled && !(e->comm && e->comm_world > 1) && !(a->options & (YKPRED_EVAL_DIRECT | YKPRED_EVAL_SPREAD_COUNT_ONLY));
  hipGraphExec_t exec = nullptr;
  if (graphable) {
    ykpred_engine::GraphKey key{e->tables_version, pre, filt, a->options, (void*)bitmap, e->last_counts, e->last_decisions, e->last_keys};
    for (size_t i = 0; i < e->graphs.size();) {
      if (e->graphs[i].first.version != e->tables_version) {
        (void)hipGraphExecDestroy(e->graphs[i].second);
        e->graphs.erase(e->graphs.begin() + (long)i);
      } else {
        if (e->graphs[i].first == key) exec = e->graphs[i].second;
        ++i;
      }
    }
    bool repeated = false;
    for (size_t i = 0; i < e->seen.size();) {
      if (e->seen[i].version != e->tables_version) {
        e->seen.erase(e->seen.begin() + (long)i);
        continue;
      }
      repeated = repeated || e->seen[i] == key;
      ++i;
    }
    if (!repeated && e->seen.size() < 8) e->seen.push_back(key);
    if (!exec && repeated) {
      hipGraph_t g = nullptr;
      int crc = YKPRED_E_DEVICE;
      if (hipStreamBeginCapture(st, hipStreamCaptureModeThreadLocal) == hipSuccess) {
        crc = enqueue();
        if (hipStreamEndCapture(st, &g) != hipSuccess) crc = YKPRED_E_DEVICE;
      }
      if (crc == YKPRED_OK && g && hipGraphInstantiate(&exec, g, nullptr, nullptr, 0) == hipSuccess) {
        if (e->graphs.size() >= 8) {
          (void)hipGraphExecDestroy(e->graphs.front().second);
          e->graphs.erase(e->graphs.begin());
        }
        e->graphs.emplace_back(key, exec);
      } else {
        exec = nullptr;
        e->graph_disabled = true;
        (void)hipGetLastError();
      }
      if (g) (void)hipGraphDestroy(g);
    }
  }
  if (exec) {
    HIPCHK(hipGraphLaunch(exec, st));
  } else {
    int rc = enqueue();
    if (rc < 0) return rc;
    if (rc == 1) {
      tm.done(st);
      return YKPRED_OK;
    }
  }
  tm.done(st);
  if (e->ev_eval_done) (void)hipEventRecord(e->ev_eval_done, st);
  e->bitmap_epoch = e->nodes_epoch;
  e->last_pre = pre;
  e->last_filt = filt;
  e->last_eval_valid = true;
  if (!(a->options & (YKPRED_EVAL_SKIP_BITMAP | YKPRED_EVAL_DIRTY_CLASSES))) e->n_full_evals++;
  if (!(a->options & (YKPRED_EVAL_SKIP_BITMAP | YKPRED_EVAL_DIRTY_CLASSES))) std::fill(e->h_row_stale.begin(), e->h_row_stale.end(), 0);
  if (want_dec) {
    e->win_partial = use_run_decide_pass;
    e->rank_valid = true;
    e->ranked_specs_version = e->specs_version;
    e->ranked_nodes_epoch = e->nodes_epoch;
    e->ranked_pre = pre;
    e->ranked_filt = filt;
    e->ranked_has_first = e->decide_skip;
  }
  e->last_has_keys = want_keys;
  return YKPRED_OK;
}

int32_t ykpred_eval_nodes(ykpred_engine_t* e, const ykpred_eval_args_t* a, int32_t num_nodes, const int32_t* node_index) {
  YK_SERIALISE(e);
  Range roctx_range("ykpred:eval_nodes");
  if (e) e->n_node_patches++;
  if (!e || !a || num_nodes < 0 || (num_nodes > 0 && !node_index)) return fail(e, YKPRED_E_INVALID, "eval_nodes: bad argument");
  HIPCHK(hipSetDevice(e->cfg.device));
  hipStream_t st = a->stream ? (hipStream_t)a->stream : e->own_stream;
  const unsigned pre = a->prefilter_plugins, filt = a->filter_plugins;
  u64* bitmap = a->bitmap ? (u64*)a->bitmap : e->d_bitmap.as<u64>();
  if (e->classes_dirty || !e->last_eval_valid || pre != e->last_pre || filt != e->last_filt || (void*)bitmap != e->last_bitmap)
    return fail(e, YKPRED_E_STATE, "eval_nodes: no matching previous ykpred_eval (tables, plugin lists or bitmap changed)");
  const bool topo = (pre & filt & (YKPRED_PLUGIN_POD_TOPOLOGY_SPREAD | YKPRED_PLUGIN_INTER_POD_AFFINITY)) && e->fam_spread.D > 0;
  const bool sharded = e->comm && e->comm_world > 1;
  const bool hist_ready = a->options & YKPRED_EVAL_SPREAD_COUNTS_READY, hist_only = a->options & YKPRED_EVAL_SPREAD_COUNT_ONLY;
  const bool topo_pass = topo && e->P > 0 && (num_nodes > 0 || sharded || hist_ready || hist_only);
  if (topo && e->spread_dirty) return fail(e, YKPRED_E_STATE, "eval_nodes: topology tables changed — run ykpred_eval");
  for (int i = 0; i < num_nodes; ++i)
    if (node_index[i] < 0 || node_index[i] >= e->N) return fail(e, YKPRED_E_INVALID, "eval_nodes: node index out of range");
  Timer tm{e, (a->options & YKPRED_EVAL_PROFILE) != 0};
  tm.start(st);
  const bool want_cnt = a->options & YKPRED_OUT_COUNTS;
  const bool want_keys = a->options & YKPRED_OUT_DECISION_KEYS;
  const bool want_dec = (a->options & YKPRED_OUT_DECISIONS) || want_keys;
  if (topo_pass) {
    const size_t cells = (size_t)std::max<int64_t>(e->spread_cells, 1) * sizeof(int), mins = (size_t)std::max(e->spread_constraints, 1) * sizeof(int);
    HIPCHK(e->d_sp_cnt_prev.ensure(cells));
    HIPCHK(e->d_sp_present_prev.ensure(cells));
    HIPCHK(e->d_sp_min_prev.ensure(mins));
    HIPCHK(e->d_sig_changed.ensure((size_t)e->fam_spread.D * sizeof(int)));
    if (e->hist_epoch == 0) return fail(e, YKPRED_E_STATE, "eval_nodes: no topology histograms from a previous ykpred_eval");
    if (!hist_ready) {
      HIPCHK(hipMemcpyAsync(e->d_sp_cnt_prev.p, e->d_sp_cnt.p, cells, hipMemcpyDeviceToDevice, st));
      HIPCHK(hipMemcpyAsync(e->d_sp_present_prev.p, e->d_sp_present.p, cells, hipMemcpyDeviceToDevice, st));
      HIPCHK(hipMemcpyAsync(e->d_sp_min_prev.p, e->d_sp_min.p, mins, hipMemcpyDeviceToDevice, st));
      TRY(run_spread_prefilter(e, st, &tm, true, false));
    }
    if (hist_only) {
      tm.done(st);
      return YKPRED_OK;
    }
    if (!hist_ready) TRY(allreduce_spread(e, st));
    TRY(run_spread_prefilter(e, st, &tm, false, true));
    e->hist_epoch = e->nodes_epoch;
    tm.begin(st);
    hipLaunchKernelGGL(ykk::k_spread_diff, dim3((unsigned)e->fam_spread.D), dim3(ykk::kWave), 0, st, spread_sigs(e), e->d_sp_cnt_prev.as<int>(),
                       e->d_sp_present_prev.as<int>(), e->d_sp_min_prev.as<int>(), e->d_sig_changed.as<int>());
    tm.end(st, "k_spread_diff");
  }
  if (num_nodes > 0 && e->P > 0) {
    std::vector<int32_t> nodes(node_index, node_index + num_nodes);
    std::sort(nodes.begin(), nodes.end());
    nodes.erase(std::unique(nodes.begin(), nodes.end()), nodes.end());
    HIPCHK(e->d_class_word.ensure((size_t)std::max(e->C, 1) * ykk::kMaxColGroups * sizeof(u64)));
    ykk::NodeTable nt = node_table(e);
    ykk::SpecTable stbl = spec_table(e);
    size_t i = 0;
    while (i < nodes.size()) {
      ykk::ColumnGroups cg{};
      int filled = 0;
      while (i < nodes.size() && cg.n_groups < ykk::kMaxColGroups && filled < 64) {
        int w = nodes[i] >> 6;
        cg.word[cg.n_groups] = w;
        cg.first[cg.n_groups] = filled;
        while (i < nodes.size() && (nodes[i] >> 6) == w && filled < 64) cg.nodes[filled++] = nodes[i++];
        cg.n_groups++;
        if (i < nodes.size() && (nodes[i] >> 6) == w) break;
      }
      cg.first[cg.n_groups] = filled;
      tm.begin(st);
      hipLaunchKernelGGL(ykk::k_column_class, dim3((unsigned)((e->C + ykk::kBlock - 1) / ykk::kBlock)), dim3(ykk::kBlock), 0, st, nt, stbl, cg,
                         e->C, e->d_class_first.as<int>(), e->d_class_pin.as<int>(), e->d_pod_spec.as<int>(), e->d_pod_row.as<int>(), pre, filt, bitmap,
                         e->row_stride, e->d_class_word.as<u64>(), e->d_class_count.as<int>());
      tm.end(st, "k_column_class");
      tm.begin(st);
      hipLaunchKernelGGL(ykk::k_column_patch, dim3((unsigned)((e->P + ykk::kBlock - 1) / ykk::kBlock)), dim3(ykk::kBlock), 0, st, cg, e->P,
                         e->d_pod_class.as<int>(), e->d_pod_row.as<int>(), e->d_class_word.as<u64>(), e->d_class_count.as<int>(), bitmap, e->row_stride,
                         want_cnt ? (int*)(a->counts ? a->counts : e->last_counts) : nullptr);
      tm.end(st, "k_column_patch");
// ... 477 lines not shown
  HIPCHK(hipMemcpyAsync(base + o_asks, asks, (size_t)n_asks * sizeof(int), hipMemcpyHostToDevice, st));
  ykk::NodeTable nt = node_table(e);
  nt.req = (const i64*)(base + o_req);
  nt.count = (const int*)(base + o_cnt);
  if (live_ports) nt.ports = (const u64*)(base + o_ports);
  ykk::ClassTable ct{e->d_class_sig.as<int>(), e->d_class_pin.as<int>(), e->d_chunk_class.as<int>(), e->d_chunk_begin.as<int>(),
                     e->d_chunk_len.as<int>(), e->d_chunk_first.as<int>(), e->d_members.as<int>(), e->d_chunk_zone.as<int>(), 0, nullptr};
  const bool spread_err = ((filt & YKPRED_PLUGIN_POD_TOPOLOGY_SPREAD) && !(pre & YKPRED_PLUGIN_POD_TOPOLOGY_SPREAD)) ||
                          ((filt & YKPRED_PLUGIN_INTER_POD_AFFINITY) && !(pre & YKPRED_PLUGIN_INTER_POD_AFFINITY)) ||
                          ((filt & YKPRED_PLUGIN_NODE_PORTS) && !(pre & YKPRED_PLUGIN_NODE_PORTS));
  ykk::RoundArgs ra{};
  ra.asks = (const int*)(base + o_asks);
  ra.pod_spec = e->d_pod_spec.as<int>();
  ra.pod_pin = e->d_pod_pin.as<int>();
  ra.pod_class = e->d_pod_class.as<int>();
  ra.perm = e->d_perm.as<int>();
  ra.rank = e->d_rank.as<int>();
  ra.key0 = e->d_key.as<u64>();
  ra.name_rank = e->has_name_rank ? e->d_name_rank.as<int>() : nullptr;
  ra.rkey = (const u64*)(base + o_rkey);
  ra.rtie = (const int*)(base + o_rtie);
  if (e->N > 0)
    hipLaunchKernelGGL(ykk::k_round_ranked_keys, dim3((unsigned)((e->N + ykk::kBlock - 1) / ykk::kBlock)), dim3(ykk::kBlock), 0, st, e->N, ra.perm, ra.key0,
                       ra.name_rank, (u64*)(base + o_rkey), (int*)(base + o_rtie));
  ra.pre = pre;
  ra.filt = filt;
  ra.row_words = e->row_words;
  ra.all_fail = spread_err ? 1 : 0;
  ra.req = (i64*)(base + o_req);
  ra.count = (int*)(base + o_cnt);
  ra.ports = live_ports ? (u64*)(base + o_ports) : nullptr;
  ra.moved_bits = (u64*)(base + o_bits);
  ra.cursor = (int*)(base + o_cur);
  ra.n_moved = (int*)(base + o_nm);
  ra.cap = (int)cap;
  ra.cap64 = (int)cap64;
  ra.slot_of = (int*)(base + o_slot);
  ra.m_node = (int*)(base + o_mnode);
  ra.m_tie = (int*)(base + o_mtie);
  ra.m_key = (u64*)(base + o_mkey);
  ra.m_free = (i64*)(base + o_mfree);
  ra.m_room = (int*)(base + o_mroom);
  ra.m_ports = (u64*)(base + o_mports);
  ra.m_taint = (u64*)(base + o_mtaint);
  ra.m_label = (u64*)(base + o_mlabel);
  ra.m_dom = (int*)(base + o_mdom);
  ra.m_flags = (unsigned*)(base + o_mflags);
  ra.dead = (u64*)(base + o_dead);
  ra.failed = keep_failed ? (u64*)(base + o_failed) : nullptr;
  ra.out = (int*)(base + o_out);
  ra.prof = e->round_prof ? (i64*)(base + o_prof) : nullptr;
  ra.mode = ykk::kRoundDecide;
  ra.node_offset = e->node_offset;
  if (fx_current) {
    ra.fx.off = e->fx_contrib ? e->d_fx_off.as<int>() : nullptr;
    ra.fx.cls = e->d_fx_cls.as<int>();
    ra.fx.cnt = e->d_fx_cnt.as<int>();
    ra.fx.occupied = (live_ports && e->fx_ports) ? e->d_fx_occ.as<u64>() : nullptr;
  }
  ykk::SpecTable stbl = spec_table(e);
  if (topo_on) {
    HIPCHK(hipMemcpyAsync(base + o_hist, e->d_sp_cnt.p, (size_t)e->spread_cells * sizeof(int), hipMemcpyDeviceToDevice, st));
    HIPCHK(hipMemcpyAsync(base + o_minv, e->d_sp_min.p, (size_t)e->spread_constraints * sizeof(int), hipMemcpyDeviceToDevice, st));
    stbl.spread.cnt = (int*)(base + o_hist);
    stbl.spread.minv = (int*)(base + o_minv);
    std::vector<int32_t> sig_of;
    for (size_t d = 0; d < e->spread_sig.size(); ++d) sig_of.insert(sig_of.end(), e->spread_sig[d].size(), (int32_t)d);
    sig_of.resize(G, 0);
    TRY(upload(e, e->d_sp_sig_of, sig_of.data(), sig_of.size(), st));
    HIPCHK(hipStreamSynchronize(st));
    ra.topo_on = 1;
    ra.G = e->spread_constraints;
    ra.sig_aff = ykk::AffSigs{e->d_sig_aff_flags.as<unsigned>(), e->d_sig_aff_off.as<int>(), e->d_sig_aff_terms.as<u64>(), e->d_sig_pre_off.as<int>(),
                              e->d_sig_pre_terms.as<u64>()};
    ra.sig_tol = e->d_sig_tol.as<u64>();
    ra.sig_of = e->d_sp_sig_of.as<int>();
    ra.mn = (int*)(base + o_mn);
    ra.at_min = (int*)(base + o_at);
    ra.nd = (int*)(base + o_nd);
    if (e->spread_constraints > 0)
      hipLaunchKernelGGL(ykk::k_round_topo_init, dim3((unsigned)e->spread_constraints), dim3(ykk::kWave), 0, st, stbl.spread, e->spread_constraints,
                         (int*)(base + o_mn), (int*)(base + o_at), (int*)(base + o_nd));
  }
  TRY(complete_windows(e, st));
  const ykk::Planes pr = ranked_planes_of(e, pre, filt, false, e->ranked_has_first);
  ra.cdesc = (const u64*)(base + o_cdesc);
  if (e->C > 0)
    hipLaunchKernelGGL(ykk::k_round_class_desc, dim3((unsigned)((e->C + ykk::kBlock - 1) / ykk::kBlock)), dim3(ykk::kBlock), 0, st, ct, pr, e->C,
                       (u64*)(base + o_cdesc));
  if (batched) {
    Rccl* r = sharded ? rccl() : nullptr;
    const int W = sharded ? e->comm_world : 1, me = sharded ? e->comm_rank : 0;
    constexpr int K = ykk::kPropK;
    auto cw_of = [](int b) { return (b * K + 63) / 64; };
    auto bytes_of = [&](int b) { return (size_t)b * K * sizeof(ykk::RoundProposal) + (size_t)b * (size_t)cw_of(b) * sizeof(u64); };
    char* d_send = base + o_prop;
    char* d_all = base + o_allprop;
    int* d_list = (int*)(base + o_list);
    int* d_nlist = d_list + kShardBatchMax * K;
    int* d_forced = (int*)(base + o_forced);
    int* d_runlen = (int*)(base + o_runlen);
    ykk::RoundNodeDelta* d_deltas = (ykk::RoundNodeDelta*)(base + o_deltas);
    std::vector<ykk::RoundNodeDelta> deltas;
    std::vector<int32_t> run_len;
    if (e->h_round_pinned_bytes < (size_t)W * kBatchBytesMax) {
      if (e->h_round_pinned) (void)hipHostFree(e->h_round_pinned);
      e->h_round_pinned = nullptr;
      e->h_round_pinned_bytes = 0;
      if (hipHostMalloc(&e->h_round_pinned, (size_t)W * kBatchBytesMax, hipHostMallocDefault) == hipSuccess) e->h_round_pinned_bytes = (size_t)W * kBatchBytesMax;
      else (void)hipGetLastError();
    }
    std::vector<char> all_pageable(e->h_round_pinned ? 0 : (size_t)W * kBatchBytesMax);
    char* const all = e->h_round_pinned ? (char*)e->h_round_pinned : all_pageable.data();
    std::vector<int32_t> forced;
    int* d_delta = (sharded && topo_on) ? (int*)(base + o_delta) : nullptr;
    int* d_alldelta = (sharded && topo_on) ? (int*)(base + o_alldelta) : nullptr;
    std::vector<int32_t> h_alldelta;
    auto spec_has_signature = [&](int spec) { return topo_on && e->spec_sig_spread[(size_t)spec] >= 0; };
    auto spec_contributes = [&](int spec) {
      return topo_on && e->fx_contrib && (size_t)spec + 1 < e->h_fx_off.size() && e->h_fx_off[(size_t)spec + 1] > e->h_fx_off[(size_t)spec];
    };
    std::vector<uint8_t> touched((size_t)std::max(e->KS, 1), 0);
    std::vector<int32_t> touched_list;
    auto touches = [&](int spec) {
      if (touched_list.empty()) return false;
      const int d = e->spec_sig_spread[(size_t)spec];
      if (d < 0 || (size_t)d >= e->spread_sig.size()) return true;
      for (const ykpred_spread_t& c : e->spread_sig[(size_t)d])
        if (c.selector_class >= 0 && c.selector_class < e->KS && touched[(size_t)c.selector_class]) return true;
      return false;
    };
    struct Accepted {
      int64_t ord;
      int64_t gnode;
      u64 key0, key1;
      i64 alloc[ykk::kMaxR], used[ykk::kMaxR];
      int room;
      int rank, node, didx;
      int pods;
      i64 add[ykk::kMaxR];
    };
    const bool fit_on = (filt & YKPRED_PLUGIN_NODE_RESOURCES_FIT) && (pre & YKPRED_PLUGIN_NODE_RESOURCES_FIT);
    auto still_fits = [&](int spec, const Accepted& n) {
      if (!fit_on) return true;
      if (n.room < 1) return false;
      for (int rr = 0; rr < e->R && rr < ykk::kMaxR; ++rr) {
        const i64 q = e->h_req[(size_t)spec * (size_t)e->R + (size_t)rr];
        if (q > 0 && q > n.alloc[rr] - n.used[rr]) return false;
      }
      return true;
    };
    auto spec_wants_ports = [&](int spec) {
      for (int kp = 0; kp < e->KP; ++kp)
        if (e->h_wanted[(size_t)spec * (size_t)e->KP + (size_t)kp] != 0) return true;
      return false;
    };
    auto less2 = [](u64 ka, int64_t oa, u64 kb, int64_t ob) { return ka < kb || (ka == kb && oa < ob); };
    struct Entry {
      u64 key;
      int64_t ord;
      int g, q;
    };
    std::vector<Accepted> acc;
    std::unordered_map<int64_t, int32_t> acc_of;
    std::vector<Entry> ents;
    const int R = e->R;
// ... 2358 lines not shown
```

### yunikorn-k8shim_amd/csrc/engine/kernels.hip.h

```cpp
#pragma once
#include <hip/hip_runtime.h>
#include <stdint.h>

#include <type_traits>

namespace ykk {

typedef unsigned long long u64;
typedef long long i64;

constexpr int kMaxR = 8;
constexpr int kMaxKT = 4;
constexpr int kMaxW = 8;
constexpr int kMaxWTotal = 32;
constexpr int kMaxKD = 8;
constexpr int kMaxKP = 4;

constexpr int kWave = 64;
constexpr int kBlock = 256;
constexpr int kWavesPerBlock = kBlock / kWave;
constexpr int kSigsPerBlock = 16;
constexpr int kSigsPerBlockMany = 64;
constexpr int kManySigs = 4096;
__host__ __device__ inline int sigs_per_block(int D) { return D > kManySigs ? kSigsPerBlockMany : kSigsPerBlock; }
// ... 1808 lines not shown
    u64 base[NIT];
    {
      const ConstRun* cr = (const ConstRun*)(unsigned long long)(runs + run);
      const int st = cr->st, sa = cr->sa, ss = cr->ss;
      const u64* p0 = pl.res + w_first + lane;
      const u64* pt = (pl.tol && st >= 0) ? pl.tol + (size_t)st * pl.stride + w_first + lane : p0;
      const u64* pa = (pl.aff && sa >= 0) ? pl.aff + (size_t)sa * pl.stride + w_first + lane : p0;
      const u64* ps = (pl.spread && ss >= 0) ? pl.spread + (size_t)ss * pl.stride + w_first + lane : p0;
#pragma unroll
      for (int it = 0; it < NIT; ++it) {
        const u64 v = p0[it * kWave] & pt[it * kWave] & pa[it * kWave] & ps[it * kWave];
        base[it] = (w_first + it * kWave + lane < rw && it < nit) ? v : 0ull;
      }
    }
    for (;;) {
      const int cls = __builtin_amdgcn_readfirstlane(da.x), dest0 = __builtin_amdgcn_readfirstlane(da.y);
      const int len = __builtin_amdgcn_readfirstlane(da.z), slots = __builtin_amdgcn_readfirstlane(da.w);
      u64 m[NIT];
      int cnt = 0;
      {
        const u64* r0 = s_stage + (slots & 255) * SW + lane;
        const u64* r1 = s_stage + ((slots >> 8) & 255) * SW + lane;
        const u64* r2 = s_stage + ((slots >> 16) & 255) * SW + lane;
        const u64* r3 = s_stage + ((slots >> 24) & 255) * SW + lane;
#pragma unroll
        for (int it = 0; it < NIT; ++it) {
          m[it] = base[it] & r0[it * kWave] & r1[it * kWave] & r2[it * kWave] & r3[it * kWave];
          cnt += __popcll(m[it]);
        }
      }
      const int pc = __builtin_amdgcn_readlane(wave_sum_lane63(cnt), 63);
      ++c;
      bool more = true;
      if (c == c1) {
        if (c < unit_end) {
          cb = c;
          if (lane < 2 * kRunsBatch) s_desc[lane] = d_nx;
          c1 = min(cb + kRunsBatch, unit_end);
          d_nx = fetch(c1);
        } else {
          u += unit_step;
          if (u >= n_units) {
            more = false;
          } else {
            cb = ub[u], unit_end = ub[u + 1];
            d_nx = fetch(cb);
            if (lane < 2 * kRunsBatch) s_desc[lane] = d_nx;
            c = cb;
            c1 = min(cb + kRunsBatch, unit_end);
            d_nx = fetch(c1);
          }
        }
      }
      if (more) da = s_desc[2 * (c - cb)], db = s_desc[2 * (c - cb) + 1];
      u64* dst = bitmap + (size_t)dest0 * row_stride + w_first + lane;
      for (int i = 0; i < len; ++i, dst += row_stride) {
#pragma unroll
        for (int it = 0; it < NIT; ++it) {
          if (it < NIT - 2) {
            dst[it * kWave] = m[it];
          } else if (it < nit) {
            if (!last_seg || it < nit - 1 || w_first + it * kWave + lane < row_stride) dst[it * kWave] = m[it];
          }
        }
      }
      if (lane == 63 && pc) atomicAdd(&class_count[cls], pc);
      if (!more) return;
      if (__builtin_amdgcn_readfirstlane(db.x) != run) break;
    }
  }
}

constexpr int kBandGroups = 256;
constexpr int kBandClasses = 4;
constexpr int kBandMaxLds = 150 * 1024;
struct BandEntry {
  int slot[kBandClasses];
  int xb[kBandClasses - 1];
  int sb[kBandClasses - 1];
  int steps, first_step;
  int n, pad;
};

__global__ __launch_bounds__(kBlock) void k_class_rows(ClassTable ct, Planes pl, const int* __restrict__ class_list, int n_list, int row_words,
                                                       int row_stride, int pin_enabled, u64* __restrict__ row_table,
                                                       int* __restrict__ class_count, const int* __restrict__ class_dirty,
                                                       const int* __restrict__ class_list_b, int n_b) {
  typedef u64 u64x2 __attribute__((ext_vector_type(2)));
  const bool all_fail = pin_enabled & 2;
  pin_enabled &= 1;
  const int k = blockIdx.x * kWavesPerBlock + threadIdx.x / kWave;
  if (k >= n_list + n_b) return;
  const bool store = k < n_list;
  const int cls = store ? class_list[k] : class_list_b[k - n_list];
  if (class_dirty && !class_dirty[cls]) return;
  const int lane = threadIdx.x % kWave;
  const int sr = ct.sig[cls * 4 + 0], st = ct.sig[cls * 4 + 1], sa = ct.sig[cls * 4 + 2], ss = ct.sig[cls * 4 + 3];
  const int pin = pin_enabled ? ct.pin[cls] : -1;
  const ClassRows cr = class_rows(pl, sr, st, sa, ss);
  u64* dst = row_table + (size_t)k * row_stride;
  int pc = 0;
  for (int w = 2 * lane; w < row_stride; w += 2 * kWave) {
    u64x2 x = {0, 0};
    if (w < row_words && pin != -2 && !all_fail) {
      x = u64x2{~0ull, ~0ull};
#pragma unroll
      for (int i = 0; i < kMaxClassRows; ++i)
        if (i < cr.n) x &= *(const u64x2*)(cr.row[i] + w);
      if (cr.ni) {
        x.x &= class_idx_word(cr, w);
        if (w + 1 < row_words) x.y &= class_idx_word(cr, w + 1);
      }
      if (w + 1 >= row_words) x.y = 0;
      if (pin >= 0) {
        x.x &= (w == (pin >> 6)) ? (1ull << (pin & 63)) : 0ull;
        x.y &= (w + 1 == (pin >> 6)) ? (1ull << (pin & 63)) : 0ull;
      }
    }
    pc += __popcll(x.x) + __popcll(x.y);
    if (store) *(u64x2*)(dst + w) = x;
  }
#pragma unroll
  for (int off = 32; off > 0; off >>= 1) pc += __shfl_down(pc, off, kWave);
  if (lane == 0) class_count[cls] = pc;
}

constexpr int kBandBlock = kBlock + kWave;
__global__ __launch_bounds__(kBandBlock) void k_expand_bands(u64* __restrict__ out, const u64* __restrict__ class_rows,
                                                             const BandEntry* __restrict__ tab, int n_bands, int row_stride) {
  typedef u64 u64x2 __attribute__((ext_vector_type(2)));
  extern __shared__ u64 band_lds[];
  const int b = blockIdx.x, tid = threadIdx.x;
  const int row_b = row_stride * 8;
  constexpr long kWin = (long)kBandGroups * 4096;
  if (tid >= kBlock) {
    const int lane = tid - kBlock;
    const int pieces = row_stride / 2;
    auto load_rows = [&](int band) {
      const BandEntry be = tab[(size_t)band * kBandGroups + b];
#pragma unroll
      for (int c = 0; c < kBandClasses; ++c) {
        if (c >= be.n && c > 0) break;
        const u64x2* src = (const u64x2*)(class_rows + (size_t)be.slot[c] * row_stride);
        u64x2* dst = (u64x2*)(band_lds + (size_t)((band & 1) * kBandClasses + c) * row_stride);
        for (int i0 = 0; i0 < pieces; i0 += 4 * kWave) {
          u64x2 r[4];
#pragma unroll
          for (int k = 0; k < 4; ++k)
            if (i0 + k * kWave + lane < pieces) r[k] = src[i0 + k * kWave + lane];
#pragma unroll
          for (int k = 0; k < 4; ++k)
            if (i0 + k * kWave + lane < pieces) dst[i0 + k * kWave + lane] = r[k];
        }
      }
    };
    load_rows(0);
    __syncthreads();
    for (int band = 0; band < n_bands; ++band) {
      if (band + 1 < n_bands) load_rows(band + 1);
      __syncthreads();
    }
    return;
  }
  __syncthreads();
  const int p = b * 4096 + tid * 16;
  const unsigned urow_b = (unsigned)row_b;
  const unsigned dcol = (unsigned)(kWin % row_b);
  unsigned ucol = (unsigned)(p % row_b);
  for (int band = 0; band < n_bands; ++band) {
    const BandEntry cur = tab[(size_t)band * kBandGroups + b];
    const int s0 = cur.first_step, s1 = s0 + cur.steps;
    const char* lds = (const char*)(band_lds + (size_t)(band & 1) * kBandClasses * row_stride);
    unsigned kb[kBandClasses - 1];
#pragma unroll
    for (int i = 0; i < kBandClasses - 1; ++i)
      kb[i] = cur.xb[i] == 0x7fffffff ? 0xffffffffu : (((unsigned)cur.xb[i] << 8) | (unsigned)(cur.sb[i] - s0));
    char* win_base = (char*)out + (long)s0 * kWin;
    auto run_band = [&](auto ncls_tag) {
      constexpr int kN = decltype(ncls_tag)::value;
      constexpr int kU = 4;
      for (int s = s0; s < s1; s += kU) {
        u64x2 v[kU];
        bool live[kU];
#pragma unroll
        for (int u = 0; u < kU; ++u) {
          unsigned off = ucol;
          live[u] = p >= (int)ucol;
          if (kN > 1) {
            const unsigned key = ((unsigned)(p - (int)ucol) << 8) | (unsigned)(s + u - s0);
#pragma unroll
            for (int i = 0; i < kN - 1; ++i) off += key >= kb[i] ? urow_b : 0u;
          }
          v[u] = *(const u64x2*)(lds + off);
          const unsigned t = ucol + dcol;
          ucol = min(t, t - urow_b);
        }
#pragma unroll
        for (int u = 0; u < kU; ++u) {
          if (live[u]) *(u64x2*)(win_base + p) = v[u];
          win_base += kWin;
        }
      }
    };
    if (cur.n <= 1)
      run_band(std::integral_constant<int, 1>{});
    else if (cur.n == 2)
      run_band(std::integral_constant<int, 2>{});
// ... 3035 lines not shown
```

Measured before the change: 40360 billion evals/s.

## Decide best node per class from class row bitmaps via sliced rank-min kernel

Adds a k_decide_rows path that computes each class's best node by taking, per node slice, the minimum rank over set bits of the class row bitmap, then picks the global minimum per class and maps it through perm. This lets decisions skip building fully ranked planes; ranked planes are marked invalid and completed lazily before rounds. The eval setup is refactored into a PlaneLaunch struct. It adds a slice_min buffer and a second pass, and correctness depends on the new ranked_valid invalidation tracking.

```diff
diff --git a/yunikorn-k8shim_amd/csrc/engine/engine.hip b/yunikorn-k8shim_amd/csrc/engine/engine.hip
--- a/yunikorn-k8shim_amd/csrc/engine/engine.hip
+++ b/yunikorn-k8shim_amd/csrc/engine/engine.hip
@@ -336,6 +336,9 @@
   uint64_t specs_version = 1, ranked_specs_version = 0, ranked_nodes_epoch = 0;
   unsigned ranked_pre = 0, ranked_filt = 0;
   bool ranked_has_first = false;
+  bool ranked_valid = false;
+  int decide_rows = 1;
+  DevBuf d_rows_min;
   DevBuf d_round;
   DevBuf d_fx_off, d_fx_cls, d_fx_cnt, d_fx_occ, d_sp_sig_of;
   uint64_t fx_version = 0;
@@ -412,6 +415,7 @@
   if (e && (code == YKPRED_E_DEVICE || code == YKPRED_E_NOMEM)) {
     e->last_eval_valid = false;
     e->rank_valid = false;
+    e->ranked_valid = false;
     e->classes_dirty = true;
     e->spread_dirty = true;
     e->hist_epoch = 0;
@@ -496,6 +500,7 @@
 
 int build_classes(ykpred_engine* e, hipStream_t st) {
   e->tables_version++;
+  e->ranked_valid = false;
   const int P = e->P;
   auto& ids = e->class_ids;
   ids.clear();
@@ -1153,6 +1158,7 @@
   for (DevBuf* b : {&e->planes_canon, &e->planes_ranked}) {
     if (b->cap < need || e->plane_rows_alloc != rows) {
       e->tables_version++;
+      e->ranked_valid = false;
       HIPCHK(b->ensure(need));
       HIPCHK(hipMemsetAsync(b->p, 0, need, st));
     }
@@ -1162,6 +1168,7 @@
   for (DevBuf* b : {&e->base_canon, &e->base_ranked}) {
     if (b->cap < base_need) {
       e->tables_version++;
+      e->ranked_valid = false;
       HIPCHK(b->ensure(base_need));
       HIPCHK(hipMemsetAsync(b->p, 0, base_need, st));
     }
@@ -1565,6 +1572,7 @@
       else if (key == "sweep_groups") e->sweep_groups = std::max(val, 0);
       else if (key == "class_runs") e->class_runs = val;
       else if (key == "run_decide") e->run_decide = val;
+      else if (key == "decide_rows") e->decide_rows = val;
       else if (key == "fuse_rows") e->fuse_rows = val;
       else if (key == "fuse_wpl") e->fuse_wpl = val;
       else if (key == "fuse_combine") e->fuse_combine = val;
@@ -1621,7 +1629,7 @@
                     &e->d_rank, &e->d_perm, &e->d_sreq, &e->d_stol, &e->d_sflags, &e->d_aff_off, &e->d_aff_terms, &e->d_pre_off,
                     &e->d_pre_terms, &e->d_dim_val, &e->d_dim_order, &e->d_dim_chunk_dim, &e->d_dim_chunk_begin, &e->d_dim_chunk_len,
                     &e->d_res_rows, &e->d_big_dim, &e->d_walk_big, &e->d_walk_begin, &e->d_walk_len, &e->d_sfree_c, &e->d_pmask_c,
-                    &e->d_sfree_r, &e->d_pmask_r, &e->d_rbits_c, &e->d_sorted, &e->d_sorted_off, &e->d_ent_c, &e->d_agree, &e->d_topo_agree, &e->d_bytes_gather, &e->d_fuse_rec, &e->d_fuse_combo_rec, &e->d_fuse_combo, &e->d_run_ranges, &e->d_no_decide, &e->d_glin_r, &e->d_run_classes, &e->d_run_units, &e->d_sweep_rows, &e->d_sweep_runs, &e->d_sweep_units, &e->d_chunk_list_b0, &e->d_walk2_order, &e->d_walk2_big, &e->d_walk2_begin, &e->d_walk2_len, &e->d_idx_c, &e->d_win_r, &e->d_pfx_r, &e->d_slice_desc, &e->d_slice_general, &e->d_chunk_list_b, &e->d_first_r, &e->d_sig_tol, &e->d_sig_tolflags, &e->d_sig_aff_flags, &e->d_sig_aff_off,
+                    &e->d_sfree_r, &e->d_pmask_r, &e->d_rbits_c, &e->d_sorted, &e->d_sorted_off, &e->d_ent_c, &e->d_agree, &e->d_topo_agree, &e->d_bytes_gather, &e->d_fuse_rec, &e->d_fuse_combo_rec, &e->d_fuse_combo, &e->d_run_ranges, &e->d_no_decide, &e->d_glin_r, &e->d_run_classes, &e->d_run_units, &e->d_sweep_rows, &e->d_sweep_runs, &e->d_sweep_units, &e->d_chunk_list_b0, &e->d_walk2_order, &e->d_walk2_big, &e->d_walk2_begin, &e->d_walk2_len, &e->d_idx_c, &e->d_win_r, &e->d_pfx_r, &e->d_slice_desc, &e->d_slice_general, &e->d_chunk_list_b, &e->d_first_r, &e->d_rows_min, &e->d_sig_tol, &e->d_sig_tolflags, &e->d_sig_aff_flags, &e->d_sig_aff_off,
                     &e->d_sig_aff_terms, &e->d_sig_pre_off, &e->d_sig_pre_terms, &e->d_pod_spec, &e->d_pod_pin, &e->d_pod_class,
                     &e->d_class_sig, &e->d_class_pin, &e->d_class_first, &e->d_class_word, &e->d_chunk_class, &e->d_chunk_begin, &e->d_chunk_len, &e->d_chunk_first,
                     &e->d_pod_row, &e->d_band_tab, &e->d_class_rows_a, &e->d_class_list_a, &e->d_class_slot_a, &e->d_fix_row, &e->d_fix_slot, &e->d_chunk_zone,
@@ -1666,6 +1674,7 @@
   HIPCHK(hipSetDevice(e->cfg.device));
   hipStream_t st = e->own_stream;
   e->rank_valid = false;
+  e->ranked_valid = false;
   const size_t N = (size_t)n->count;
   TRY(upload(e, e->d_alloc, n->allocatable, N * (size_t)e->R, st));
   TRY(upload(e, e->d_req, n->requested, N * (size_t)e->R, st));
@@ -1725,6 +1734,7 @@
   HIPCHK(hipSetDevice(e->cfg.device));
   hipStream_t st = e->own_stream;
   e->rank_valid = false;
+  e->ranked_valid = false;
   const size_t N = (size_t)e->N;
   for (int r = 0; r < e->R; ++r) {
     HIPCHK(hipMemcpyAsync(e->d_alloc.as<i64>() + (size_t)r * N + idx, n->allocatable + r, sizeof(i64), hipMemcpyHostToDevice, st));
@@ -1772,6 +1782,7 @@
   if (e) e->tables_version++;
   if (e) e->ask_epoch++;
   if (e) e->specs_version++;
+  if (e) e->ranked_valid = false;
   if (!e || !s || s->count < 0) return fail(e, YKPRED_E_INVALID, "set_specs: bad argument");
   if (s->count > 0 && (!s->requests || !s->tolerated || !s->flags || !s->aff_term_off || !s->pre_term_off))
     return fail(e, YKPRED_E_INVALID, "set_specs: null column");
@@ -2090,190 +2101,39 @@
   return YKPRED_OK;
 }
 
-static int validate_state(ykpred_engine* e) {
-  if (!e->nodes_set || !e->specs_set || !e->pods_set) return fail(e, YKPRED_E_STATE, "nodes, specs and pods must be uploaded first");
-  for (int p = 0; p < e->P; ++p) {
-    int s = e->h_pod_spec[(size_t)p], pin = e->h_pod_pin[(size_t)p];
-    if (s < 0 || s >= e->S) return fail(e, YKPRED_E_INVALID, "pod references a spec that was not uploaded");
-    if (pin < YKPRED_UNKNOWN_NODE_NAME || pin >= e->N) return fail(e, YKPRED_E_INVALID, "pod node_name_index out of range");
-  }
-  return YKPRED_OK;
-}
-
-int32_t ykpred_eval(ykpred_engine_t* e, const ykpred_eval_args_t* a) {
-  YK_SERIALISE(e);
-  Range roctx_range("ykpred:eval");
-  if (!e || !a) return fail(e, YKPRED_E_INVALID, "eval: bad argument");
-  HIPCHK(hipSetDevice(e->cfg.device));
-  hipStream_t st = a->stream ? (hipStream_t)a->stream : e->own_stream;
-  if (e->classes_dirty) {
-    if (a->options & (YKPRED_EVAL_SKIP_BITMAP | YKPRED_EVAL_DIRTY_CLASSES))
-      return fail(e, YKPRED_E_STATE, "eval: the pod classes are due for a rebuild — run a full ykpred_eval (bitmap included)");
-    TRY(validate_state(e));
-    TRY(build_classes(e, e->own_stream));
-  }
-  const unsigned pre = a->prefilter_plugins, filt = a->filter_plugins;
-  const bool spread_filt = filt & YKPRED_PLUGIN_POD_TOPOLOGY_SPREAD, spread_pre = pre & YKPRED_PLUGIN_POD_TOPOLOGY_SPREAD;
-  const bool ipa_filt = filt & YKPRED_PLUGIN_INTER_POD_AFFINITY, ipa_pre = pre & YKPRED_PLUGIN_INTER_POD_AFFINITY;
-  const bool spread_err = (spread_filt && !spread_pre) || (ipa_filt && !ipa_pre) ||
-                          ((filt & YKPRED_PLUGIN_NODE_PORTS) && !(pre & YKPRED_PLUGIN_NODE_PORTS));
-  if (e->spread_dirty) TRY(build_spread_tables(e, e->own_stream));
-  const bool pts_en = spread_filt && spread_pre, ipa_en = ipa_filt && ipa_pre;
-  const bool spread_on = (pts_en || ipa_en) && e->fam_spread.D > 0;
-  const int N = e->N, P = e->P;
-  const size_t bitmap_bytes = (size_t)std::max(std::max(e->rows_total, e->row_capacity), 1) * (size_t)e->row_stride * sizeof(u64);
-  u64* bitmap = (u64*)a->bitmap;
-  int64_t bitmap_rows = 0;
-  if (!bitmap || (void*)bitmap == e->d_bitmap.p) {
-    HIPCHK(e->d_bitmap.ensure(bitmap_bytes));
-    bitmap = e->d_bitmap.as<u64>();
-    bitmap_rows = (int64_t)(e->d_bitmap.cap / ((size_t)std::max(e->row_stride, 1) * sizeof(u64)));
-  } else {
-    bitmap_rows = a->bitmap_rows ? (int64_t)a->bitmap_rows : (int64_t)e->row_capacity;
-    if (bitmap_rows == 0)
-      return fail(e, YKPRED_E_INVALID, "eval: a caller-owned bitmap needs eval_args.bitmap_rows or ykpred_set_row_capacity (it must hold layout.num_rows rows)");
-    if ((int64_t)e->rows_total > bitmap_rows)
-      return fail(e, YKPRED_E_INVALID, "eval: the caller-owned bitmap holds fewer rows than the layout needs (layout.num_rows)");
-  }
-  e->last_bitmap = bitmap;
-  e->last_bitmap_rows = bitmap_rows;
-  HIPCHK(e->d_counts.ensure((size_t)std::max(P, 1) * sizeof(int)));
-  HIPCHK(e->d_decisions.ensure((size_t)std::max(P, 1) * sizeof(int)));
-  HIPCHK(e->d_keys.ensure((size_t)std::max(P, 1) * sizeof(i64)));
-  e->last_counts = a->counts ? a->counts : e->d_counts.p;
-  e->last_decisions = a->decisions ? a->decisions : e->d_decisions.p;
-  e->last_keys = a->decision_keys ? a->decision_keys : e->d_keys.p;
-  TRY(ensure_planes(e, st));
-  if (e->n_big > 0) {
-    const size_t cells = (size_t)e->n_big * (size_t)std::max(e->row_words, 1);
-    for (DevBuf* b : {&e->d_sfree_c, &e->d_sfree_r}) HIPCHK(b->ensure(cells * 64 * sizeof(i64)));
-    for (DevBuf* b : {&e->d_pmask_c, &e->d_pmask_r}) HIPCHK(b->ensure(cells * 65 * sizeof(u64)));
-    HIPCHK(e->d_rbits_c.ensure(cells * ykk::kRankBits * sizeof(u64)));
-    HIPCHK(e->d_ent_c.ensure(cells * 65 * sizeof(unsigned)));
-    HIPCHK(e->d_glin_r.ensure(cells * 65 * sizeof(unsigned)));
-    const int idx_stride_before = e->idx_stride;
-    e->idx_stride = (std::max(e->row_words, e->row_stride) + 63) / 64 * 64;
-    for (DevBuf* b : {&e->d_idx_c}) {
-      const size_t need = (size_t)e->fam_res.D * (size_t)e->idx_stride;
-      if (b->cap < need || !b->p || idx_stride_before != e->idx_stride) {
-        HIPCHK(b->ensure(need));
-        HIPCHK(hipMemsetAsync(b->p, 64, need, st));
-      }
-    }
-    {
-      const size_t need = (size_t)e->fam_res.D * 64;
-      if (e->d_win_r.cap < need || !e->d_win_r.p) {
-        HIPCHK(e->d_win_r.ensure(need));
-        HIPCHK(hipMemsetAsync(e->d_win_r.p, 64, need, st));
-      }
-    }
-  }
-  Timer tm{e, (a->options & YKPRED_EVAL_PROFILE) != 0};
-  tm.start(st);
-  if (N == 0 || P == 0) {
-    tm.done(st);
-    return YKPRED_OK;
-  }
-  ykk::NodeTable nt = node_table(e);
-  const bool want_keys = a->options & YKPRED_OUT_DECISION_KEYS;
-  const bool want_dec = (a->options & YKPRED_OUT_DECISIONS) || want_keys;
-  const bool want_cnt = a->options & YKPRED_OUT_COUNTS;
-  const int nblk_nodes = (N + ykk::kBlock - 1) / ykk::kBlock;
-
-  bool use_run_decide_pass = false;
-  auto enqueue = [&]() -> int {
-  if (spread_on || (a->options & YKPRED_EVAL_SPREAD_COUNT_ONLY)) {
-    const bool ready = a->options & YKPRED_EVAL_SPREAD_COUNTS_READY, only = a->options & YKPRED_EVAL_SPREAD_COUNT_ONLY;
-    TRY(run_spread_prefilter(e, st, &tm, !ready, false));
-    if (only) return 1;
-    if (!ready) TRY(allreduce_spread(e, st));
-    TRY(run_spread_prefilter(e, st, &tm, false, true));
-    e->hist_epoch = e->nodes_epoch;
-  }
-  if (a->options & YKPRED_EVAL_DIRECT) {
-    ykk::SpecTable stbl = spec_table(e);
-    dim3 grid((unsigned)((P + ykk::kWave - 1) / ykk::kWave), (unsigned)((e->row_stride + ykk::kWavesPerBlock - 1) / ykk::kWavesPerBlock));
-    tm.begin(st);
-    hipLaunchKernelGGL(ykk::k_direct, grid, dim3(ykk::kBlock), 0, st, nt, stbl, P, e->d_pod_spec.as<int>(), e->d_pod_pin.as<int>(),
-                       e->d_pod_row.as<int>(), pre, filt, bitmap, e->row_words, e->row_stride);
-    tm.end(st, "k_direct");
-    HIPCHK(hipGetLastError());
-    return 1;
-  }
-
-  const unsigned wgroups = (unsigned)((e->row_words + ykk::kWavesPerBlock - 1) / ykk::kWavesPerBlock);
-  const bool res_on = filt & YKPRED_PLUGIN_NODE_RESOURCES_FIT;
-  const bool aff_on = (filt | pre) & YKPRED_PLUGIN_NODE_AFFINITY;
-  const int fit_error = (pre & YKPRED_PLUGIN_NODE_RESOURCES_FIT) ? 0 : 1;
-  auto sig_chunks = [](int D) {
+struct PlaneLaunch {
+  ykpred_engine* e;
+  Timer* tm;
+  unsigned pre, filt;
+  bool spread_on, pts_en, ipa_en;
+  int* first_r;
+  bool use_sweep = false, sweep_rows_on = false, use_run_decide = false;
+  ykk::NodeTable nt{};
+  ykk::AffSigs as{};
+  ykk::PlaneOut o_res{}, o_tol{}, o_aff{}, o_spread{};
+  unsigned wgroups = 0;
+  bool res_on = false, aff_on = false;
+  int fit_error = 0;
+  PlaneLaunch(ykpred_engine* e_, Timer* tm_, unsigned pre_, unsigned filt_, bool spread_on_, bool pts_en_, bool ipa_en_, int* first_r_)
+      : e(e_), tm(tm_), pre(pre_), filt(filt_), spread_on(spread_on_), pts_en(pts_en_), ipa_en(ipa_en_), first_r(first_r_) {
+    nt = node_table(e);
+    as = ykk::AffSigs{e->d_sig_aff_flags.as<unsigned>(), e->d_sig_aff_off.as<int>(), e->d_sig_aff_terms.as<u64>(), e->d_sig_pre_off.as<int>(),
+                      e->d_sig_pre_terms.as<u64>()};
+    auto out_of = [&](const Family& f) {
+      return ykk::PlaneOut{e->planes_canon.as<u64>() + (size_t)f.base * e->row_stride, e->planes_ranked.as<u64>() + (size_t)f.base * e->row_stride,
+                           e->row_stride, f.D, nullptr};
+    };
+    o_res = out_of(e->fam_res), o_tol = out_of(e->fam_tol), o_aff = out_of(e->fam_aff), o_spread = out_of(e->fam_spread);
+    wgroups = (unsigned)((e->row_words + ykk::kWavesPerBlock - 1) / ykk::kWavesPerBlock);
+    res_on = filt & YKPRED_PLUGIN_NODE_RESOURCES_FIT;
+    aff_on = (filt | pre) & YKPRED_PLUGIN_NODE_AFFINITY;
+    fit_error = (pre & YKPRED_PLUGIN_NODE_RESOURCES_FIT) ? 0 : 1;
+  }
+  static unsigned sig_chunks(int D) {
     const int spb = ykk::sigs_per_block(D);
     return (unsigned)((D + spb - 1) / spb);
-  };
-  ykk::AffSigs as{e->d_sig_aff_flags.as<unsigned>(), e->d_sig_aff_off.as<int>(), e->d_sig_aff_terms.as<u64>(), e->d_sig_pre_off.as<int>(),
-                  e->d_sig_pre_terms.as<u64>()};
-  auto canon_of = [&](const Family& f) { return e->planes_canon.as<u64>() + (size_t)f.base * e->row_stride; };
-  auto ranked_of = [&](const Family& f) { return e->planes_ranked.as<u64>() + (size_t)f.base * e->row_stride; };
-  ykk::PlaneOut o_res{canon_of(e->fam_res), ranked_of(e->fam_res), e->row_stride, e->fam_res.D, nullptr};
-  ykk::PlaneOut o_tol{canon_of(e->fam_tol), ranked_of(e->fam_tol), e->row_stride, e->fam_tol.D, nullptr};
-  ykk::PlaneOut o_aff{canon_of(e->fam_aff), ranked_of(e->fam_aff), e->row_stride, e->fam_aff.D, nullptr};
-  ykk::PlaneOut o_spread{canon_of(e->fam_spread), ranked_of(e->fam_spread), e->row_stride, e->fam_spread.D, nullptr};
-  const bool full_pass = !(a->options & (YKPRED_EVAL_SKIP_BITMAP | YKPRED_EVAL_DIRTY_CLASSES));
-  const bool counts_early_here = e->early_counts != 0 && full_pass && e->n_classes_a > 0 && e->patch_chunks == 0 &&
-                                 !((long)e->NC * e->wave_combine_below > (long)P) && e->n_classes_b <= 16384;
-  const bool zero_counts_beside = full_pass && !counts_early_here && e->ev_zero != nullptr && e->C >= 65536 &&
-                                  (a->options & (YKPRED_OUT_DECISIONS | YKPRED_OUT_DECISION_KEYS)) != 0;
-  const bool use_sweep = e->sweep_ready && e->sweep_runs > 0 && res_on && !fit_error && full_pass && !counts_early_here;
-  const bool sweep_rows_on = use_sweep && e->n_big > 0 && e->sweep_row_off[ykk::kMaxIdxRows] > 0;
-  const bool fuse_on = e->fuse_ready && res_on && !fit_error && full_pass && !counts_early_here && aff_on && !spread_err;
-  const bool use_run_decide = e->run_decide != 0 && e->sweep_ready && e->run_ranges > 0 && res_on && !fit_error && e->n_big > 0 &&
-                              (a->options & (YKPRED_OUT_DECISIONS | YKPRED_OUT_DECISION_KEYS)) && e->walk2_chunks >= 0 &&
-                              e->C == e->run_decide_classes;
-  use_run_decide_pass = use_run_decide;
-  ykk::ClassTable ct{e->d_class_sig.as<int>(), e->d_class_pin.as<int>(),  e->d_chunk_class.as<int>(), e->d_chunk_begin.as<int>(),
-                     e->d_chunk_len.as<int>(), e->d_chunk_first.as<int>(), e->d_members.as<int>(), e->d_chunk_zone.as<int>(), (use_sweep ? 1 : 0) | (fuse_on ? 2 : 0),
-                     use_run_decide ? e->d_no_decide.as<int>() : nullptr};
-  ykk::Planes pc{res_on ? o_res.canon : nullptr, o_tol.canon, aff_on ? o_aff.canon : nullptr, spread_on ? o_spread.canon : nullptr,
-                 e->row_stride, e->d_res_rows.as<int>(), 1 + e->R, e->d_idx_c.as<unsigned char>(), e->idx_stride, e->d_pmask_c.as<u64>(), e->row_words,
-                 nullptr, 0, 0, 0, 0, 0, nullptr, nullptr, nullptr, nullptr, nullptr};
-  int* first_r = nullptr;
-  if ((a->options & (YKPRED_OUT_DECISIONS | YKPRED_OUT_DECISION_KEYS)) && e->decide_skip) {
-    HIPCHK(e->d_first_r.ensure((size_t)std::max(e->plane_rows_alloc, 1) * sizeof(int)));
-    first_r = e->d_first_r.as<int>();
-  }
-  if (want_dec && res_on && e->n_big > 0 && !fit_error) HIPCHK(e->d_pfx_r.ensure((size_t)e->n_big * (size_t)std::max(e->row_words, 1) * sizeof(i64)));
-  ykk::Planes pr = ranked_planes_of(e, pre, filt, spread_on, first_r != nullptr);
-  pc.n_big = pr.n_big;
-  pc.rbits = e->d_rbits_c.as<u64>();
-  const int pin_on = ((filt & YKPRED_PLUGIN_NODE_NAME) ? 1 : 0) | (spread_err ? 2 : 0);
-  hipStream_t sb = e->aux_stream;
-
-  if (want_dec) {
-    HIPCHK(hipEventRecord(e->ev_fork, st));
-    HIPCHK(hipStreamWaitEvent(sb, e->ev_fork, 0));
-    if (zero_counts_beside) {
-      HIPCHK(hipMemsetAsync(e->d_class_count.p, 0, (size_t)e->C * sizeof(int), sb));
-      HIPCHK(hipEventRecord(e->ev_zero, sb));
-    }
-    if (first_r) HIPCHK(hipMemsetAsync(first_r, 0x7f, (size_t)std::max(e->plane_rows_alloc, 1) * sizeof(int), sb));
-    tm.begin(sb);
-    hipLaunchKernelGGL(ykk::k_score, dim3((unsigned)nblk_nodes), dim3(ykk::kBlock), 0, sb, nt, e->d_score.as<double>(), e->d_key.as<u64>());
-    tm.end(sb, "k_score");
-    int* hist = e->d_rankbuf.as<int>();
-    int* bucket_off = hist + ykk::kRankBuckets;
-    int* cursor = bucket_off + ykk::kRankBuckets + 1;
-    int* members = cursor + ykk::kRankBuckets;
-    HIPCHK(hipMemsetAsync(hist, 0, ykk::kRankBuckets * sizeof(int), sb));
-    tm.begin(sb);
-    hipLaunchKernelGGL(ykk::k_rank_hist, dim3((unsigned)nblk_nodes), dim3(ykk::kBlock), 0, sb, N, e->d_score.as<double>(), hist);
-    hipLaunchKernelGGL(ykk::k_rank_scan, dim3(1), dim3(ykk::kRankBuckets), 0, sb, hist, bucket_off, cursor);
-    hipLaunchKernelGGL(ykk::k_rank_fill, dim3((unsigned)nblk_nodes), dim3(ykk::kBlock), 0, sb, N, e->d_score.as<double>(), e->d_key.as<u64>(),
-                       e->has_name_rank ? e->d_name_rank.as<int>() : (const int*)nullptr, cursor, members, e->d_member_tie.as<int>(),
-                       e->d_member_key.as<u64>());
-    hipLaunchKernelGGL(ykk::k_rank_final, dim3((unsigned)ykk::kRankBuckets), dim3(ykk::kBlock), 0, sb, bucket_off, members,
-                       e->d_member_tie.as<int>(), e->d_member_key.as<u64>(), e->d_rank.as<int>(), e->d_perm.as<int>());
-    tm.end(sb, "k_rank");
-  }
-  auto base_of = [&](DevBuf& buf) {
+  }
+  ykk::BasePlanes base_of(DevBuf& buf) const {
     ykk::BasePlanes bp;
     bp.req = buf.as<u64>();
     bp.taint = bp.req + (size_t)64 * e->W * e->row_stride;
@@ -2282,14 +2142,14 @@
     bp.exists = bp.unsched + e->row_stride;
     bp.stride = e->row_stride;
     return bp;
-  };
-  auto launch_dictionary_planes = [&](hipStream_t s, const int* perm, bool ranked, const char* base_name, const char* sig_name, bool base_done = false) -> int {
+  }
+  int dictionary_planes(hipStream_t s, const int* perm, bool ranked, const char* base_name, const char* sig_name, bool base_done = false) {
     ykk::BasePlanes bp = base_of(ranked ? e->base_ranked : e->base_canon);
     if (!base_done) {
-      tm.begin(s);
+      tm->begin(s);
       hipLaunchKernelGGL(ykk::k_base_planes, dim3((unsigned)(e->W + e->KT + e->KP + 1), wgroups), dim3(ykk::kBlock), 0, s, nt, perm, bp,
                          e->row_words);
-      tm.end(s, base_name);
+      tm->end(s, base_name);
     }
     ykk::SigPlaneArgs sa{};
     sa.base = bp;
@@ -2313,7 +2173,7 @@
     sa.pre_mask = pre;
     sa.filt_mask = filt;
     sa.n_words = e->row_words;
-    tm.begin(s);
+    tm->begin(s);
     const int wpl = e->sig_wpl > 0 ? e->sig_wpl : (e->row_words >= 4 * ykk::kWave ? 4 : (e->row_words >= 2 * ykk::kWave ? 2 : 1));
     const unsigned chunks = std::max((unsigned)((std::max(sa.tol.D, sa.aff.D) + ykk::kBitSigsPerBlock - 1) / ykk::kBitSigsPerBlock), 1u);
     const unsigned ygroups = (unsigned)((e->row_words + ykk::kBlock * wpl - 1) / (ykk::kBlock * wpl));
@@ -2323,12 +2183,10 @@
       hipLaunchKernelGGL(ykk::k_sig_planes<2>, dim3(chunks, ygroups, 2u), dim3(ykk::kBlock), 0, s, sa);
     else
       hipLaunchKernelGGL(ykk::k_sig_planes<1>, dim3(chunks, ygroups, 2u), dim3(ykk::kBlock), 0, s, sa);
-    tm.end(s, sig_name);
+    tm->end(s, sig_name);
     return YKPRED_OK;
-  };
-  if (want_dec) TRY(launch_dictionary_planes(sb, e->d_perm.as<int>(), true, "k_base_planes(ranked)", "k_sig_planes(ranked)"));
-  auto ranked_walk = [](const int* perm) { return perm != nullptr; };
-  auto launch_ballot_planes = [&](hipStream_t s, const int* perm, const char* name, bool with_base = false) {
+  }
+  void ballot_planes(hipStream_t s, const int* perm, const char* name, bool with_base = false) {
     ykk::PlaneArgs pa{};
     pa.perm = perm;
     pa.res = o_res;
@@ -2346,7 +2204,7 @@
     pa.spread_en = pts_en ? 1 : 0;
     pa.ipa_en = ipa_en ? 1 : 0;
     unsigned xchunks = std::max((unsigned)pa.dims.n_chunks, sig_chunks(pa.spread.D));
-    tm.begin(s);
+    tm->begin(s);
     if (with_base) {
       xchunks = std::max(xchunks, (unsigned)(e->W + e->KT + e->KP + 1));
       hipLaunchKernelGGL(ykk::k_node_planes, dim3(std::max(xchunks, 1u), wgroups, 3u), dim3(ykk::kBlock), 0, s, nt, pa,
@@ -2354,7 +2212,7 @@
     } else {
       hipLaunchKernelGGL(ykk::k_planes, dim3(std::max(xchunks, 1u), wgroups, spread_on ? 2u : 1u), dim3(ykk::kBlock), 0, s, nt, pa);
     }
-    tm.end(s, name);
+    tm->end(s, name);
     if (res_on && e->n_big > 0 && !fit_error) {
       const bool ranked = perm != nullptr;
       ykk::DimWalk dw{e->d_dim_val.as<i64>(), e->d_dim_order.as<int>(), e->d_big_dim.as<int>(), e->d_walk_big.as<int>(), e->d_walk_begin.as<int>(),
@@ -2362,10 +2220,10 @@
                       e->n_big, e->walk_chunks, e->row_words, ranked ? nullptr : e->d_rbits_c.as<u64>(),
                       (!ranked && sweep_rows_on) ? e->d_ent_c.as<unsigned>() : nullptr, e->d_sorted.as<i64>(), e->d_sorted_off.as<int>(),
                       (ranked && use_run_decide) ? e->d_glin_r.as<unsigned>() : nullptr};
-      tm.begin(s);
+      tm->begin(s);
       hipLaunchKernelGGL(ykk::k_dim_sort, dim3((unsigned)e->n_big, wgroups), dim3(ykk::kBlock), 0, s, nt, perm, dw);
-      tm.end(s, ranked ? "k_dim_sort(ranked)" : "k_dim_sort");
-      tm.begin(s);
+      tm->end(s, ranked ? "k_dim_sort(ranked)" : "k_dim_sort");
+      tm->begin(s);
       const unsigned walk_gy = (unsigned)((e->row_words + ykk::kBlock * ykk::kWalkWords - 1) / (ykk::kBlock * ykk::kWalkWords));
       const dim3 walk_grid((unsigned)e->walk_chunks, walk_gy);
       if (!ranked && use_sweep && e->walk2_chunks >= 0) {
@@ -2396,28 +2254,246 @@
           hipLaunchKernelGGL(ykk::k_dim_walk_window<ykk::kWalkBatch>, walk_grid, dim3(ykk::kBlock), 0, s, dw, e->d_pfx_r.as<i64>(), e->d_win_r.as<unsigned char>());
         }
       }
-      tm.end(s, ranked ? "k_dim_walk(ranked)" : "k_dim_walk");
+      tm->end(s, ranked ? "k_dim_walk(ranked)" : "k_dim_walk");
     } else if (res_on && e->n_big > 0) {
-      if (!ranked_walk(perm)) (void)hipMemsetAsync(e->d_idx_c.p, 64, (size_t)e->fam_res.D * (size_t)e->idx_stride, s);
-      (void)hipMemsetAsync((ranked_walk(perm) ? e->d_pmask_r : e->d_pmask_c).p, 0, (size_t)e->n_big * (size_t)e->row_words * 65 * sizeof(u64), s);
-      if (!ranked_walk(perm)) (void)hipMemsetAsync(e->d_rbits_c.p, 0, (size_t)e->n_big * (size_t)e->row_words * ykk::kRankBits * sizeof(u64), s);
-    }
-  };
+      if (!(perm != nullptr)) (void)hipMemsetAsync(e->d_idx_c.p, 64, (size_t)e->fam_res.D * (size_t)e->idx_stride, s);
+      (void)hipMemsetAsync(((perm != nullptr) ? e->d_pmask_r : e->d_pmask_c).p, 0, (size_t)e->n_big * (size_t)e->row_words * 65 * sizeof(u64), s);
+      if (!(perm != nullptr)) (void)hipMemsetAsync(e->d_rbits_c.p, 0, (size_t)e->n_big * (size_t)e->row_words * ykk::kRankBits * sizeof(u64), s);
+    }
+  }
+  void ranked_ballot_planes(hipStream_t s) {
+    const int ballot_rows = e->fam_tol.base;
+    if (ballot_rows <= ykk::kManySigs && e->n_big == 0) {
+      tm->begin(s);
+      hipLaunchKernelGGL(ykk::k_permute_planes, dim3(sig_chunks(ballot_rows), wgroups), dim3(ykk::kBlock), 0, s, e->N, e->d_perm.as<int>(),
+                         e->planes_canon.as<u64>(), e->planes_ranked.as<u64>(), e->row_stride, ballot_rows, e->row_words, first_r);
+      tm->end(s, "k_permute_planes");
+    } else if (res_on || spread_on) {
+      ballot_planes(s, e->d_perm.as<int>(), "k_planes(ranked)");
+    }
+  }
+  int ranked_planes(hipStream_t s) {
+    if (first_r) HIPCHK(hipMemsetAsync(first_r, 0x7f, (size_t)std::max(e->plane_rows_alloc, 1) * sizeof(int), s));
+    TRY(dictionary_planes(s, e->d_perm.as<int>(), true, "k_base_planes(ranked)", "k_sig_planes(ranked)"));
+    ranked_ballot_planes(s);
+    return YKPRED_OK;
+  }
+};
+
+int complete_ranked_planes(ykpred_engine* e, hipStream_t st, unsigned pre, unsigned filt) {
+  if (e->ranked_valid) return YKPRED_OK;
+  const bool pts_en = (filt & YKPRED_PLUGIN_POD_TOPOLOGY_SPREAD) && (pre & YKPRED_PLUGIN_POD_TOPOLOGY_SPREAD);
+  const bool ipa_en = (filt & YKPRED_PLUGIN_INTER_POD_AFFINITY) && (pre & YKPRED_PLUGIN_INTER_POD_AFFINITY);
+  const bool spread_on = (pts_en || ipa_en) && e->fam_spread.D > 0;
+  int* first_r = nullptr;
+  if (e->decide_skip) {
+    HIPCHK(e->d_first_r.ensure((size_t)std::max(e->plane_rows_alloc, 1) * sizeof(int)));
+    first_r = e->d_first_r.as<int>();
+  }
+  if ((filt & YKPRED_PLUGIN_NODE_RESOURCES_FIT) && e->n_big > 0 && (pre & YKPRED_PLUGIN_NODE_RESOURCES_FIT))
+    HIPCHK(e->d_pfx_r.ensure((size_t)e->n_big * (size_t)std::max(e->row_words, 1) * sizeof(i64)));
+  Timer tm{e, false};
+  PlaneLaunch pl(e, &tm, pre, filt, spread_on, pts_en, ipa_en, first_r);
+  TRY(pl.ranked_planes(st));
+  HIPCHK(hipGetLastError());
+  e->win_partial = false;
+  e->ranked_has_first = first_r != nullptr;
+  e->ranked_valid = true;
+  return YKPRED_OK;
+}
+
+static int validate_state(ykpred_engine* e) {
+  if (!e->nodes_set || !e->specs_set || !e->pods_set) return fail(e, YKPRED_E_STATE, "nodes, specs and pods must be uploaded first");
+  for (int p = 0; p < e->P; ++p) {
+    int s = e->h_pod_spec[(size_t)p], pin = e->h_pod_pin[(size_t)p];
+    if (s < 0 || s >= e->S) return fail(e, YKPRED_E_INVALID, "pod references a spec that was not uploaded");
+    if (pin < YKPRED_UNKNOWN_NODE_NAME || pin >= e->N) return fail(e, YKPRED_E_INVALID, "pod node_name_index out of range");
+  }
+  return YKPRED_OK;
+}
+
+int32_t ykpred_eval(ykpred_engine_t* e, const ykpred_eval_args_t* a) {
+  YK_SERIALISE(e);
+  Range roctx_range("ykpred:eval");
+  if (!e || !a) return fail(e, YKPRED_E_INVALID, "eval: bad argument");
+  HIPCHK(hipSetDevice(e->cfg.device));
+  hipStream_t st = a->stream ? (hipStream_t)a->stream : e->own_stream;
+  if (e->classes_dirty) {
+    if (a->options & (YKPRED_EVAL_SKIP_BITMAP | YKPRED_EVAL_DIRTY_CLASSES))
+      return fail(e, YKPRED_E_STATE, "eval: the pod classes are due for a rebuild — run a full ykpred_eval (bitmap included)");
+    TRY(validate_state(e));
+    TRY(build_classes(e, e->own_stream));
+  }
+  const unsigned pre = a->prefilter_plugins, filt = a->filter_plugins;
+  const bool spread_filt = filt & YKPRED_PLUGIN_POD_TOPOLOGY_SPREAD, spread_pre = pre & YKPRED_PLUGIN_POD_TOPOLOGY_SPREAD;
+  const bool ipa_filt = filt & YKPRED_PLUGIN_INTER_POD_AFFINITY, ipa_pre = pre & YKPRED_PLUGIN_INTER_POD_AFFINITY;
+  const bool spread_err = (spread_filt && !spread_pre) || (ipa_filt && !ipa_pre) ||
+                          ((filt & YKPRED_PLUGIN_NODE_PORTS) && !(pre & YKPRED_PLUGIN_NODE_PORTS));
+  if (e->spread_dirty) TRY(build_spread_tables(e, e->own_stream));
+  const bool pts_en = spread_filt && spread_pre, ipa_en = ipa_filt && ipa_pre;
+  const bool spread_on = (pts_en || ipa_en) && e->fam_spread.D > 0;
+  const int N = e->N, P = e->P;
+  const size_t bitmap_bytes = (size_t)std::max(std::max(e->rows_total, e->row_capacity), 1) * (size_t)e->row_stride * sizeof(u64);
+  u64* bitmap = (u64*)a->bitmap;
+  int64_t bitmap_rows = 0;
+  if (!bitmap || (void*)bitmap == e->d_bitmap.p) {
+    HIPCHK(e->d_bitmap.ensure(bitmap_bytes));
+    bitmap = e->d_bitmap.as<u64>();
+    bitmap_rows = (int64_t)(e->d_bitmap.cap / ((size_t)std::max(e->row_stride, 1) * sizeof(u64)));
+  } else {
+    bitmap_rows = a->bitmap_rows ? (int64_t)a->bitmap_rows : (int64_t)e->row_capacity;
+    if (bitmap_rows == 0)
+      return fail(e, YKPRED_E_INVALID, "eval: a caller-owned bitmap needs eval_args.bitmap_rows or ykpred_set_row_capacity (it must hold layout.num_rows rows)");
+    if ((int64_t)e->rows_total > bitmap_rows)
+      return fail(e, YKPRED_E_INVALID, "eval: the caller-owned bitmap holds fewer rows than the layout needs (layout.num_rows)");
+  }
+  e->last_bitmap = bitmap;
+  e->last_bitmap_rows = bitmap_rows;
+  HIPCHK(e->d_counts.ensure((size_t)std::max(P, 1) * sizeof(int)));
+  HIPCHK(e->d_decisions.ensure((size_t)std::max(P, 1) * sizeof(int)));
+  HIPCHK(e->d_keys.ensure((size_t)std::max(P, 1) * sizeof(i64)));
+  e->last_counts = a->counts ? a->counts : e->d_counts.p;
+  e->last_decisions = a->decisions ? a->decisions : e->d_decisions.p;
+  e->last_keys = a->decision_keys ? a->decision_keys : e->d_keys.p;
+  TRY(ensure_planes(e, st));
+  if (e->n_big > 0) {
+    const size_t cells = (size_t)e->n_big * (size_t)std::max(e->row_words, 1);
+    for (DevBuf* b : {&e->d_sfree_c, &e->d_sfree_r}) HIPCHK(b->ensure(cells * 64 * sizeof(i64)));
+    for (DevBuf* b : {&e->d_pmask_c, &e->d_pmask_r}) HIPCHK(b->ensure(cells * 65 * sizeof(u64)));
+    HIPCHK(e->d_rbits_c.ensure(cells * ykk::kRankBits * sizeof(u64)));
+    HIPCHK(e->d_ent_c.ensure(cells * 65 * sizeof(unsigned)));
+    HIPCHK(e->d_glin_r.ensure(cells * 65 * sizeof(unsigned)));
+    const int idx_stride_before = e->idx_stride;
+    e->idx_stride = (std::max(e->row_words, e->row_stride) + 63) / 64 * 64;
+    for (DevBuf* b : {&e->d_idx_c}) {
+      const size_t need = (size_t)e->fam_res.D * (size_t)e->idx_stride;
+      if (b->cap < need || !b->p || idx_stride_before != e->idx_stride) {
+        HIPCHK(b->ensure(need));
+        HIPCHK(hipMemsetAsync(b->p, 64, need, st));
+      }
+    }
+    {
+      const size_t need = (size_t)e->fam_res.D * 64;
+      if (e->d_win_r.cap < need || !e->d_win_r.p) {
+        HIPCHK(e->d_win_r.ensure(need));
+        HIPCHK(hipMemsetAsync(e->d_win_r.p, 64, need, st));
+      }
+    }
+  }
+  Timer tm{e, (a->options & YKPRED_EVAL_PROFILE) != 0};
+  tm.start(st);
+  if (N == 0 || P == 0) {
+    tm.done(st);
+    return YKPRED_OK;
+  }
+  ykk::NodeTable nt = node_table(e);
+  const bool want_keys = a->options & YKPRED_OUT_DECISION_KEYS;
+  const bool want_dec = (a->options & YKPRED_OUT_DECISIONS) || want_keys;
+  const bool want_cnt = a->options & YKPRED_OUT_COUNTS;
+  const int nblk_nodes = (N + ykk::kBlock - 1) / ykk::kBlock;
+
+  bool use_run_decide_pass = false;
+  const bool decide_rows_pass = e->decide_rows != 0 && want_dec && e->n_big == 0 && !(a->options & (YKPRED_EVAL_SKIP_BITMAP | YKPRED_EVAL_DIRTY_CLASSES)) &&
+                                e->early_counts != 0 && e->n_classes_a > 0 && e->patch_chunks == 0 && !((long)e->NC * e->wave_combine_below > (long)P) &&
+                                e->n_classes_b <= 16384 && e->n_classes_a + e->n_classes_b == e->C;
+  const int decide_slices = (N + ykk::kDecideSliceNodes - 1) / ykk::kDecideSliceNodes;
+  if (decide_rows_pass) HIPCHK(e->d_rows_min.ensure((size_t)decide_slices * (size_t)e->C * sizeof(int)));
+  auto enqueue = [&]() -> int {
+  if (spread_on || (a->options & YKPRED_EVAL_SPREAD_COUNT_ONLY)) {
+    const bool ready = a->options & YKPRED_EVAL_SPREAD_COUNTS_READY, only = a->options & YKPRED_EVAL_SPREAD_COUNT_ONLY;
+    TRY(run_spread_prefilter(e, st, &tm, !ready, false));
+    if (only) return 1;
+    if (!ready) TRY(allreduce_spread(e, st));
+    TRY(run_spread_prefilter(e, st, &tm, false, true));
+    e->hist_epoch = e->nodes_epoch;
+  }
+  if (a->options & YKPRED_EVAL_DIRECT) {
+    ykk::SpecTable stbl = spec_table(e);
+    dim3 grid((unsigned)((P + ykk::kWave - 1) / ykk::kWave), (unsigned)((e->row_stride + ykk::kWavesPerBlock - 1) / ykk::kWavesPerBlock));
+    tm.begin(st);
+    hipLaunchKernelGGL(ykk::k_direct, grid, dim3(ykk::kBlock), 0, st, nt, stbl, P, e->d_pod_spec.as<int>(), e->d_pod_pin.as<int>(),
+                       e->d_pod_row.as<int>(), pre, filt, bitmap, e->row_words, e->row_stride);
+    tm.end(st, "k_direct");
+    HIPCHK(hipGetLastError());
+    return 1;
+  }
+
+  const bool res_on = filt & YKPRED_PLUGIN_NODE_RESOURCES_FIT;
+  const bool aff_on = (filt | pre) & YKPRED_PLUGIN_NODE_AFFINITY;
+  const int fit_error = (pre & YKPRED_PLUGIN_NODE_RESOURCES_FIT) ? 0 : 1;
+  auto canon_of = [&](const Family& f) { return e->planes_canon.as<u64>() + (size_t)f.base * e->row_stride; };
+  auto ranked_of = [&](const Family& f) { return e->planes_ranked.as<u64>() + (size_t)f.base * e->row_stride; };
+  ykk::PlaneOut o_res{canon_of(e->fam_res), ranked_of(e->fam_res), e->row_stride, e->fam_res.D, nullptr};
+  ykk::PlaneOut o_tol{canon_of(e->fam_tol), ranked_of(e->fam_tol), e->row_stride, e->fam_tol.D, nullptr};
+  ykk::PlaneOut o_aff{canon_of(e->fam_aff), ranked_of(e->fam_aff), e->row_stride, e->fam_aff.D, nullptr};
+  ykk::PlaneOut o_spread{canon_of(e->fam_spread), ranked_of(e->fam_spread), e->row_stride, e->fam_spread.D, nullptr};
+  const bool full_pass = !(a->options & (YKPRED_EVAL_SKIP_BITMAP | YKPRED_EVAL_DIRTY_CLASSES));
+  const bool counts_early_here = e->early_counts != 0 && full_pass && e->n_classes_a > 0 && e->patch_chunks == 0 &&
+                                 !((long)e->NC * e->wave_combine_below > (long)P) && e->n_classes_b <= 16384;
+  const bool zero_counts_beside = full_pass && !counts_early_here && e->ev_zero != nullptr && e->C >= 65536 &&
+                                  (a->options & (YKPRED_OUT_DECISIONS | YKPRED_OUT_DECISION_KEYS)) != 0;
+  const bool use_sweep = e->sweep_ready && e->sweep_runs > 0 && res_on && !fit_error && full_pass && !counts_early_here;
+  const bool sweep_rows_on = use_sweep && e->n_big > 0 && e->sweep_row_off[ykk::kMaxIdxRows] > 0;
+  const bool fuse_on = e->fuse_ready && res_on && !fit_error && full_pass && !counts_early_here && aff_on && !spread_err;
+  const bool use_run_decide = e->run_decide != 0 && e->sweep_ready && e->run_ranges > 0 && res_on && !fit_error && e->n_big > 0 &&
+                              (a->options & (YKPRED_OUT_DECISIONS | YKPRED_OUT_DECISION_KEYS)) && e->walk2_chunks >= 0 &&
+                              e->C == e->run_decide_classes;
+  use_run_decide_pass = use_run_decide;
+  const bool decide_from_rows = decide_rows_pass;
+  ykk::ClassTable ct{e->d_class_sig.as<int>(), e->d_class_pin.as<int>(),  e->d_chunk_class.as<int>(), e->d_chunk_begin.as<int>(),
+                     e->d_chunk_len.as<int>(), e->d_chunk_first.as<int>(), e->d_members.as<int>(), e->d_chunk_zone.as<int>(), (use_sweep ? 1 : 0) | (fuse_on ? 2 : 0),
+                     use_run_decide ? e->d_no_decide.as<int>() : nullptr};
+  ykk::Planes pc{res_on ? o_res.canon : nullptr, o_tol.canon, aff_on ? o_aff.canon : nullptr, spread_on ? o_spread.canon : nullptr,
+                 e->row_stride, e->d_res_rows.as<int>(), 1 + e->R, e->d_idx_c.as<unsigned char>(), e->idx_stride, e->d_pmask_c.as<u64>(), e->row_words,
+                 nullptr, 0, 0, 0, 0, 0, nullptr, nullptr, nullptr, nullptr, nullptr};
+  int* first_r = nullptr;
+  if ((a->options & (YKPRED_OUT_DECISIONS | YKPRED_OUT_DECISION_KEYS)) && e->decide_skip) {
+    HIPCHK(e->d_first_r.ensure((size_t)std::max(e->plane_rows_alloc, 1) * sizeof(int)));
+    first_r = e->d_first_r.as<int>();
+  }
+  if (want_dec && res_on && e->n_big > 0 && !fit_error) HIPCHK(e->d_pfx_r.ensure((size_t)e->n_big * (size_t)std::max(e->row_words, 1) * sizeof(i64)));
+  ykk::Planes pr = ranked_planes_of(e, pre, filt, spread_on, first_r != nullptr);
+  pc.n_big = pr.n_big;
+  pc.rbits = e->d_rbits_c.as<u64>();
+  const int pin_on = ((filt & YKPRED_PLUGIN_NODE_NAME) ? 1 : 0) | (spread_err ? 2 : 0);
+  hipStream_t sb = e->aux_stream;
+  PlaneLaunch planes(e, &tm, pre, filt, spread_on, pts_en, ipa_en, first_r);
+  planes.use_sweep = use_sweep, planes.sweep_rows_on = sweep_rows_on, planes.use_run_decide = use_run_decide;
+
+  if (want_dec) {
+    HIPCHK(hipEventRecord(e->ev_fork, st));
+    HIPCHK(hipStreamWaitEvent(sb, e->ev_fork, 0));
+    if (zero_counts_beside) {
+      HIPCHK(hipMemsetAsync(e->d_class_count.p, 0, (size_t)e->C * sizeof(int), sb));
+      HIPCHK(hipEventRecord(e->ev_zero, sb));
+    }
+    if (first_r && !decide_from_rows) HIPCHK(hipMemsetAsync(first_r, 0x7f, (size_t)std::max(e->plane_rows_alloc, 1) * sizeof(int), sb));
+    tm.begin(sb);
+    hipLaunchKernelGGL(ykk::k_score, dim3((unsigned)nblk_nodes), dim3(ykk::kBlock), 0, sb, nt, e->d_score.as<double>(), e->d_key.as<u64>());
+    tm.end(sb, "k_score");
+    int* hist = e->d_rankbuf.as<int>();
+    int* bucket_off = hist + ykk::kRankBuckets;
+    int* cursor = bucket_off + ykk::kRankBuckets + 1;
+    int* members = cursor + ykk::kRankBuckets;
+    HIPCHK(hipMemsetAsync(hist, 0, ykk::kRankBuckets * sizeof(int), sb));
+    tm.begin(sb);
+    hipLaunchKernelGGL(ykk::k_rank_hist, dim3((unsigned)nblk_nodes), dim3(ykk::kBlock), 0, sb, N, e->d_score.as<double>(), hist);
+    hipLaunchKernelGGL(ykk::k_rank_scan, dim3(1), dim3(ykk::kRankBuckets), 0, sb, hist, bucket_off, cursor);
+    hipLaunchKernelGGL(ykk::k_rank_fill, dim3((unsigned)nblk_nodes), dim3(ykk::kBlock), 0, sb, N, e->d_score.as<double>(), e->d_key.as<u64>(),
+                       e->has_name_rank ? e->d_name_rank.as<int>() : (const int*)nullptr, cursor, members, e->d_member_tie.as<int>(),
+                       e->d_member_key.as<u64>());
+    hipLaunchKernelGGL(ykk::k_rank_final, dim3((unsigned)ykk::kRankBuckets), dim3(ykk::kBlock), 0, sb, bucket_off, members,
+                       e->d_member_tie.as<int>(), e->d_member_key.as<u64>(), e->d_rank.as<int>(), e->d_perm.as<int>());
+    tm.end(sb, "k_rank");
+  }
+  if (want_dec && !decide_from_rows) TRY(planes.dictionary_planes(sb, e->d_perm.as<int>(), true, "k_base_planes(ranked)", "k_sig_planes(ranked)"));
   const bool fused_planes = res_on || spread_on;
-  if (fused_planes) launch_ballot_planes(st, nullptr, "k_planes+k_base_planes", true);
-  TRY(launch_dictionary_planes(st, nullptr, false, "k_base_planes", "k_sig_planes", fused_planes));
-  if (want_dec) {
+  if (fused_planes) planes.ballot_planes(st, nullptr, "k_planes+k_base_planes", true);
+  TRY(planes.dictionary_planes(st, nullptr, false, "k_base_planes", "k_sig_planes", fused_planes));
+  if (want_dec && !decide_from_rows) {
     HIPCHK(hipEventRecord(e->ev_planes, st));
     HIPCHK(hipStreamWaitEvent(sb, e->ev_planes, 0));
-    const int ballot_rows = e->fam_tol.base;
-    if (ballot_rows <= ykk::kManySigs && e->n_big == 0) {
-      tm.begin(sb);
-      hipLaunchKernelGGL(ykk::k_permute_planes, dim3(sig_chunks(ballot_rows), wgroups), dim3(ykk::kBlock), 0, sb, N, e->d_perm.as<int>(),
-                         e->planes_canon.as<u64>(), e->planes_ranked.as<u64>(), e->row_stride, ballot_rows, e->row_words, first_r);
-      tm.end(sb, "k_permute_planes");
-    } else if (res_on || spread_on) {
-      launch_ballot_planes(sb, e->d_perm.as<int>(), "k_planes(ranked)");
-    }
+    planes.ranked_ballot_planes(sb);
     if (use_run_decide) {
       tm.begin(sb);
       hipLaunchKernelGGL(ykk::k_run_decide, dim3((unsigned)((e->run_ranges + ykk::kWavesPerBlock - 1) / ykk::kWavesPerBlock)), dim3(ykk::kBlock), 0, sb, pr,
@@ -2475,6 +2551,21 @@
       if (counts_early && want_dec) {
         HIPCHK(hipEventRecord(e->ev_counts, st));
         HIPCHK(hipStreamWaitEvent(sb, e->ev_counts, 0));
+        if (decide_from_rows) {
+          const int n_tasks = e->n_classes_a + e->n_classes_b;
+          const int n_slices = decide_slices;
+          const int want_groups = std::max(1, (2 * e->num_cus + n_slices - 1) / n_slices);
+          const int per_group = std::min(ykk::kWavesPerBlock * ykk::kDecideTasksPerWave, std::max(ykk::kWavesPerBlock, (n_tasks + want_groups - 1) / want_groups));
+          const int groups = (n_tasks + per_group - 1) / per_group;
+          tm.begin(sb);
+          hipLaunchKernelGGL(ykk::k_decide_rows, dim3((unsigned)groups, (unsigned)n_slices), dim3(ykk::kBlock), 0, sb, ct, pc, e->d_class_list_a.as<int>(),
+                             e->n_classes_a, e->d_class_list_b.as<int>(), e->n_classes_b, e->row_words, e->row_stride, pin_on,
+                             e->d_class_rows_a.as<u64>(), e->d_class_count.as<int>(), e->d_rank.as<int>(), N, per_group, e->d_rows_min.as<int>(), e->decide_rows == 2 ? 0 : 1);
+          hipLaunchKernelGGL(ykk::k_decide_rows_pick, dim3((unsigned)((n_tasks + ykk::kBlock - 1) / ykk::kBlock)), dim3(ykk::kBlock), 0, sb,
+                             e->d_class_list_a.as<int>(), e->n_classes_a, e->d_class_list_b.as<int>(), e->n_classes_b, e->d_rows_min.as<int>(), n_slices,
+                             e->d_perm.as<int>(), N, e->d_class_best.as<int>());
+          tm.end(sb, "k_decide_rows");
+        }
         tm.begin(sb);
         hipLaunchKernelGGL(ykk::k_scatter, dim3((unsigned)((P + ykk::kBlock - 1) / ykk::kBlock)), dim3(ykk::kBlock), 0, sb, P,
                            e->d_pod_class.as<int>(), e->d_class_count.as<int>(), e->d_class_best.as<int>(), e->d_key.as<u64>(),
@@ -2746,7 +2837,8 @@
     e->ranked_nodes_epoch = e->nodes_epoch;
     e->ranked_pre = pre;
     e->ranked_filt = filt;
-    e->ranked_has_first = e->decide_skip;
+    if (!decide_rows_pass) e->ranked_has_first = e->decide_skip;
+    e->ranked_valid = !decide_rows_pass;
   }
   e->last_has_keys = want_keys;
   return YKPRED_OK;
@@ -3390,6 +3482,7 @@
       hipLaunchKernelGGL(ykk::k_round_topo_init, dim3((unsigned)e->spread_constraints), dim3(ykk::kWave), 0, st, stbl.spread, e->spread_constraints,
                          (int*)(base + o_mn), (int*)(base + o_at), (int*)(base + o_nd));
   }
+  TRY(complete_ranked_planes(e, st, pre, filt));
   TRY(complete_windows(e, st));
   const ykk::Planes pr = ranked_planes_of(e, pre, filt, false, e->ranked_has_first);
   ra.cdesc = (const u64*)(base + o_cdesc);
diff --git a/yunikorn-k8shim_amd/csrc/engine/kernels.hip.h b/yunikorn-k8shim_amd/csrc/engine/kernels.hip.h
--- a/yunikorn-k8shim_amd/csrc/engine/kernels.hip.h
+++ b/yunikorn-k8shim_amd/csrc/engine/kernels.hip.h
@@ -1914,6 +1914,27 @@
   int n, pad;
 };
 
+typedef u64 u64x2_t __attribute__((ext_vector_type(2)));
+__device__ __forceinline__ u64x2_t class_row_pair(const ClassRows& cr, int w, int row_words, int pin, bool all_fail) {
+  u64x2_t x = {0, 0};
+  if (w < row_words && pin != -2 && !all_fail) {
+    x = u64x2_t{~0ull, ~0ull};
+#pragma unroll
+    for (int i = 0; i < kMaxClassRows; ++i)
+      if (i < cr.n) x &= *(const u64x2_t*)(cr.row[i] + w);
+    if (cr.ni) {
+      x.x &= class_idx_word(cr, w);
+      if (w + 1 < row_words) x.y &= class_idx_word(cr, w + 1);
+    }
+    if (w + 1 >= row_words) x.y = 0;
+    if (pin >= 0) {
+      x.x &= (w == (pin >> 6)) ? (1ull << (pin & 63)) : 0ull;
+      x.y &= (w + 1 == (pin >> 6)) ? (1ull << (pin & 63)) : 0ull;
+    }
+  }
+  return x;
+}
+
 __global__ __launch_bounds__(kBlock) void k_class_rows(ClassTable ct, Planes pl, const int* __restrict__ class_list, int n_list, int row_words,
                                                        int row_stride, int pin_enabled, u64* __restrict__ row_table,
                                                        int* __restrict__ class_count, const int* __restrict__ class_dirty,
@@ -1933,28 +1954,93 @@
   u64* dst = row_table + (size_t)k * row_stride;
   int pc = 0;
   for (int w = 2 * lane; w < row_stride; w += 2 * kWave) {
-    u64x2 x = {0, 0};
-    if (w < row_words && pin != -2 && !all_fail) {
-      x = u64x2{~0ull, ~0ull};
-#pragma unroll
-      for (int i = 0; i < kMaxClassRows; ++i)
-        if (i < cr.n) x &= *(const u64x2*)(cr.row[i] + w);
-      if (cr.ni) {
-        x.x &= class_idx_word(cr, w);
-        if (w + 1 < row_words) x.y &= class_idx_word(cr, w + 1);
-      }
-      if (w + 1 >= row_words) x.y = 0;
-      if (pin >= 0) {
-        x.x &= (w == (pin >> 6)) ? (1ull << (pin & 63)) : 0ull;
-        x.y &= (w + 1 == (pin >> 6)) ? (1ull << (pin & 63)) : 0ull;
-      }
-    }
+    const u64x2 x = class_row_pair(cr, w, row_words, pin, all_fail);
     pc += __popcll(x.x) + __popcll(x.y);
     if (store) *(u64x2*)(dst + w) = x;
   }
 #pragma unroll
   for (int off = 32; off > 0; off >>= 1) pc += __shfl_down(pc, off, kWave);
   if (lane == 0) class_count[cls] = pc;
+}
+
+constexpr int kDecideSliceWords = kWave;
+constexpr int kDecideSliceNodes = kDecideSliceWords * 64;
+constexpr int kDecideTasksPerWave = 16;
+__global__ __launch_bounds__(kBlock) void k_decide_rows(ClassTable ct, Planes pl, const int* __restrict__ class_list, int n_list,
+                                                        const int* __restrict__ class_list_b, int n_b, int row_words, int row_stride, int pin_enabled,
+                                                        const u64* __restrict__ row_table, const int* __restrict__ class_count,
+                                                        const int* __restrict__ rank, int n_nodes, int tasks_per_group, int* __restrict__ slice_min, int staged) {
+  __shared__ int s_rank[kDecideSliceNodes];
+  const int n_tasks = n_list + n_b;
+  const int slice = blockIdx.y, node0 = slice * kDecideSliceNodes;
+  const int lane = threadIdx.x % kWave, wave = threadIdx.x / kWave;
+  const int w = slice * kDecideSliceWords + lane;
+  const int k_first = blockIdx.x * tasks_per_group + wave, k_end = min(n_tasks, (int)(blockIdx.x + 1) * tasks_per_group);
+  __shared__ u64 s_x[kWavesPerBlock][kDecideTasksPerWave][kWave];
+  {
+    u64 xs[kDecideTasksPerWave];
+#pragma unroll
+    for (int t = 0; t < kDecideTasksPerWave; ++t) {
+      const int k = k_first + t * kWavesPerBlock;
+      xs[t] = (k < k_end && k < n_list && w < row_words) ? row_table[(size_t)k * row_stride + w] : 0;
+    }
+#pragma unroll
+    for (int t = 0; t < kDecideTasksPerWave; ++t) s_x[wave][t][lane] = xs[t];
+  }
+  int r[kDecideSliceWords];
+  if (staged) {
+    for (int i = threadIdx.x; i < kDecideSliceNodes; i += kBlock) s_rank[i] = node0 + i < n_nodes ? rank[node0 + i] : kNoWord;
+    __syncthreads();
+#pragma unroll
+    for (int j = 0; j < kDecideSliceWords; ++j) r[j] = s_rank[j * 64 + lane];
+  } else {
+#pragma unroll
+    for (int j = 0; j < kDecideSliceWords; ++j) r[j] = node0 + j * 64 + lane < n_nodes ? rank[node0 + j * 64 + lane] : kNoWord;
+  }
+  const bool all_fail = pin_enabled & 2;
+  const unsigned my_bit = 1u << (lane & 31);
+  const bool upper = lane >= 32;
+#pragma unroll 1
+  for (int t = 0; t < kDecideTasksPerWave; ++t) {
+    const int k = k_first + t * kWavesPerBlock;
+    if (k >= k_end) break;
+    int best = kNoWord;
+    {
+      u64 x = s_x[wave][t][lane];
+      if (k >= n_list) {
+        const int cls = class_list_b[k - n_list];
+        if (class_count[cls] > 0) {
+          const int pin = (pin_enabled & 1) ? ct.pin[cls] : -1;
+          const ClassRows cr = class_rows(pl, ct.sig[cls * 4 + 0], ct.sig[cls * 4 + 1], ct.sig[cls * 4 + 2], ct.sig[cls * 4 + 3]);
+          const u64x2_t p = class_row_pair(cr, w & ~1, row_words, pin, all_fail);
+          x = (w & 1) ? p.y : p.x;
+        }
+      }
+      if (__ballot(x != 0)) {
+        const unsigned xlo = (unsigned)x, xhi = (unsigned)(x >> 32);
+#pragma unroll
+        for (int j = 0; j < kDecideSliceWords; ++j) {
+          const unsigned lo = (unsigned)__builtin_amdgcn_readlane((int)xlo, j), hi = (unsigned)__builtin_amdgcn_readlane((int)xhi, j);
+          if ((lo | hi) == 0) continue;
+          if ((upper ? hi : lo) & my_bit) best = min(best, r[j]);
+        }
+#pragma unroll
+        for (int off = 32; off > 0; off >>= 1) best = min(best, __shfl_xor(best, off, kWave));
+      }
+    }
+    if (lane == 0) slice_min[(size_t)slice * n_tasks + k] = best;
+  }
+}
+__global__ __launch_bounds__(kBlock) void k_decide_rows_pick(const int* __restrict__ class_list, int n_list, const int* __restrict__ class_list_b,
+                                                             int n_b, const int* __restrict__ slice_min, int n_slices,
+                                                             const int* __restrict__ perm, int n_nodes, int* __restrict__ class_best) {
+  const int n_tasks = n_list + n_b;
+  const int k = blockIdx.x * kBlock + threadIdx.x;
+  if (k >= n_tasks) return;
+  int best = kNoWord;
+  for (int s = 0; s < n_slices; ++s) best = min(best, slice_min[(size_t)s * n_tasks + k]);
+  const int cls = k < n_list ? class_list[k] : class_list_b[k - n_list];
+  class_best[cls] = (best >= 0 && best < n_nodes) ? perm[best] : -1;
 }
 
 constexpr int kBandBlock = kBlock + kWave;
```

Measured after the change: 41020 billion evals/s (median of 6 runs). +1.7%, better.
